# cheneeheng/2s-AGCN

Measured on AMD Instinct MI355X. Metric: skeleton-clips/sec fwd+bwd, NTU (N,3,300,25,2), higher is better.
Workload: dtype f32; 1 GPU; AGCN joint-stream NTU-xview shape, full training step (fwd, CE, bwd, grad all-reduce, clip 1.0, SGD nesterov); per_gpu_batch=64, global_batch=64, input=(N,3,300,25,2), parallelism=dp1, bn=per-replica

## Files before the change

### 2s-agcn_amd/csrc/conv_gemm_bf16.hip

```cpp
#include "agcn_common.h"
#include "epilogue.h"
#include "gate.h"
#include "split_f16.h"

namespace {

typedef __bf16 bf16x8 __attribute__((ext_vector_type(8)));
typedef __bf16 bf16x2 __attribute__((ext_vector_type(2)));
typedef float f32x2 __attribute__((ext_vector_type(2)));
typedef unsigned u32x4 __attribute__((ext_vector_type(4)));
typedef f32x4 f32x4_u __attribute__((aligned(4)));

constexpr int CK = 16, NW = 8, NT = 512;

struct BfArgs {
  const float* in;
  const unsigned short* wp;
  const float* bias;
  float* out;
  float* stats;
  const float* add1;
  const float* mask1;
  const float* add2;
  const float* mask2;
  int N, M, Kinner, in_rows;
  int V, T_src, T_out, tt, ntiles;
  int src_stride, f_off;
  int out_fs, out_fo, T_full;
  int FW, WLR;
  int accumulate;
  int nchunks, nmb;
  int off_b;
  int off_bias;
  int dbg;
  int relu;
  const float* in_absmax;
};

struct GateBfArgs : BfArgs {
  GateArgs gate;
  int off_gate;
};
template <bool GATE> struct BfArgsOf { typedef BfArgs type; };
template <> struct BfArgsOf<true> { typedef GateBfArgs type; };

struct BfPackArgs {
  const float* w;
  unsigned short* wp;
  int M, Kinner, nchunks;
  long sa_m, sa_c;
  int tap_mul, tap_add, tap_flip_from;
};

__device__ __forceinline__ unsigned pack_bf16(float a, float b) {
  f32x2 v = {a, b};
  bf16x2 p = __builtin_convertvector(v, bf16x2);
  return __builtin_bit_cast(unsigned, p);
}
__device__ __forceinline__ float lo_as_f32(unsigned p) { return __builtin_bit_cast(float, p << 16); }
__device__ __forceinline__ float hi_as_f32(unsigned p) { return __builtin_bit_cast(float, p & 0xffff0000u); }

__device__ __forceinline__ void split_pair(float a, float b, unsigned& ph, unsigned& pm, unsigned& pl) {
  ph = pack_bf16(a, b);
  const float ra = a - lo_as_f32(ph), rb = b - hi_as_f32(ph);
  pm = pack_bf16(ra, rb);
  pl = pack_bf16(ra - lo_as_f32(pm), rb - hi_as_f32(pm));
}

template <bool F16>
__device__ __forceinline__ f32x16 mfma_split(bf16x8 x, bf16x8 y, f32x16 c) {
  if constexpr (F16)
    return __builtin_amdgcn_mfma_f32_32x32x16_f16(__builtin_bit_cast(f16x8, x), __builtin_bit_cast(f16x8, y), c, 0, 0, 0);
  else
    return __builtin_amdgcn_mfma_f32_32x32x16_bf16(x, y, c, 0, 0, 0);
}

template <int TAPS, int BM, bool F16 = false>
__global__ void __launch_bounds__(256) pack_weights_bf16_kernel(const BfPackArgs p) {
  constexpr int PER_PLANE = TAPS * 2 * BM * 8;
  const int ch = blockIdx.x % p.nchunks, mb = blockIdx.x / p.nchunks;
  unsigned short* dst = p.wp + (long)blockIdx.x * 3 * PER_PLANE;
  for (int e = threadIdx.x; e < PER_PLANE / 2; e += 256) {
    const int j = (e & 3) * 2;
    const int ml = (e >> 2) % BM;
    const int r = (e >> 2) / BM;
    const int h = r & 1, tap = r >> 1;
    const int m = mb * BM + ml;
    const int gt = p.tap_flip_from >= 0 ? (p.tap_flip_from - (tap * p.tap_mul + p.tap_add)) : tap;
    float v[2];
#pragma unroll
    for (int q = 0; q < 2; ++q) {
      const int kc = ch * CK + h * 8 + j + q;
      v[q] = (m < p.M && kc < p.Kinner) ? p.w[(long)m * p.sa_m + (long)kc * p.sa_c + gt] : 0.f;
    }
    unsigned ph, pm, pl = 0;
    if constexpr (F16) split_pair_f16(v[0] * F16_W_SCALE, v[1] * F16_W_SCALE, ph, pm);
    else split_pair(v[0], v[1], ph, pm, pl);
    const int o = ((tap * 2 + h) * BM + ml) * 8 + j;
    *reinterpret_cast<unsigned*>(dst + 0 * PER_PLANE + o) = ph;
    *reinterpret_cast<unsigned*>(dst + 1 * PER_PLANE + o) = pm;
    *reinterpret_cast<unsigned*>(dst + 2 * PER_PLANE + o) = pl;
  }
}

template <int TAPS, int NPL, int WQ, int TM, int TN = 1, bool F16 = false, bool GATE = false>
__global__ void __launch_bounds__(NT, (TAPS == 1 && TM == 2 && TN == 1) ? 4 : 2) conv_gemm_bf16_kernel(const typename BfArgsOf<GATE>::type a) {
  constexpr int BM = TM * 32;
  constexpr int A_PLANE = TAPS * 2 * BM * 16;
  constexpr int A4 = NPL * A_PLANE / 16;
  constexpr int EA = (A4 + NT - 1) / NT;
  extern __shared__ __attribute__((aligned(16))) unsigned char smem[];
  unsigned char* Ab = smem;
  unsigned char* Bb = smem + a.off_b;

  const int tid = threadIdx.x, lane = tid & 63;
  const int wave = __builtin_amdgcn_readfirstlane(tid >> 6);
  const int lr = lane & 31, h = lane >> 5;
  const int bid = xcd_remap(blockIdx.x, gridDim.x);
  const int mbk = bid % a.nmb;
  const int nt_id = bid / a.nmb;
  const int n = nt_id / a.ntiles, tile_id = nt_id - n * a.ntiles;
  const int m0 = mbk * BM;
  const int V = a.V, tt = a.tt, t0 = tile_id * tt;
  const int ttv = tt * V;
  const int nvalid = min(tt, a.T_out - t0) * V;
  const int Psrc = a.T_src * V;
  const int f0 = t0 * a.src_stride + a.f_off;
  const int WL = a.FW * V, WLR = a.WLR;
  const int g0 = f0 * V;
  float rs_s = 1.f, rs_inv = 1.f;
  if constexpr (F16) { f16_range_scale(a.in_absmax, rs_s, rs_inv); rs_inv *= F16_W_INV; }

  int boff[TN];
#pragma unroll
  for (int tn = 0; tn < TN; ++tn) {
    int q = (wave * TN + tn) * 32 + lr;
    if (q >= ttv) q = 0;
    const int tl = q / V;
    boff[tn] = tl * a.src_stride * V + (q - tl * V);
  }

  float* bias_s = reinterpret_cast<float*>(smem + a.off_bias);
  for (int e = tid; e < BM; e += NT) bias_s[e] = (a.bias && m0 + e < a.M) ? a.bias[m0 + e] : 0.f;

  f32x16 acc[TM][TN];
#pragma unroll
  for (int tm = 0; tm < TM; ++tm)
#pragma unroll
    for (int tn = 0; tn < TN; ++tn)
#pragma unroll
      for (int j = 0; j < 16; ++j) acc[tm][tn][j] = 0.f;

  const int hb = wave & 1, wq = wave >> 1;
  const int qlen = (WL + 3) >> 2;
  u32x4 ra[EA];
  float rb[WQ][8];
  const int KP = a.nchunks * CK;
  const float* gl = nullptr;
  float gpos[WQ];
  if constexpr (GATE) {
    gl = reinterpret_cast<const float*>(smem + a.off_gate);
    gate_stage<NT>(reinterpret_cast<float*>(smem + a.off_gate), a.gate, n, V, a.T_src, a.Kinner, f0, a.FW, KP);
    __syncthreads();
#pragma unroll
    for (int u = 0; u < WQ; ++u) {
      const int rr = lane + 64 * u;
      gpos[u] = rr < qlen ? gate_pos(gl, KP, wq * qlen + rr, V, WL) : 0.f;
    }
    if constexpr (F16) {
      if (a.in_absmax) {
        f16_range_scale_of<14>(*a.in_absmax * gate_bound(gl, KP, a.FW, lane), rs_s, rs_inv);
        rs_inv *= F16_W_INV;
      }
    }
  }
  const u32x4* wp4 = reinterpret_cast<const u32x4*>(a.wp) + (long)mbk * a.nchunks * (3 * A_PLANE / 16);

  auto issue_loads = [&](int ch) __attribute__((always_inline)) {
    const u32x4* src = wp4 + (long)ch * (3 * A_PLANE / 16);
#pragma unroll
    for (int u = 0; u < EA; ++u) ra[u] = src[min(tid + u * NT, A4 - 1)];
    const int kc0 = ch * CK + hb * 8;
#pragma unroll
    for (int u = 0; u < WQ; ++u) {
      const int rr = lane + 64 * u;
      const int r = wq * qlen + rr;
      const int gp = g0 + r;
      const bool okp = rr < qlen && r < WL && gp >= 0 && gp < Psrc;
#pragma unroll
      for (int c = 0; c < 8; ++c) {
        const bool ok = okp && (kc0 + c) < a.Kinner;
        rb[u][c] = a.in[((long)n * a.in_rows + (ok ? (kc0 + c) : 0)) * Psrc + (ok ? gp : 0)];
      }
    }
  };
  auto commit_lds = [&](int ch) __attribute__((always_inline)) {
#pragma unroll
    for (int u = 0; u < EA; ++u)
      if (tid + u * NT < A4) reinterpret_cast<u32x4*>(Ab)[tid + u * NT] = ra[u];
    const int kc0 = ch * CK + hb * 8;
#pragma unroll
    for (int u = 0; u < WQ; ++u) {
      const int rr = lane + 64 * u;
      const int r = wq * qlen + rr;
      const int gp = g0 + r;
      const bool okp = rr < qlen && r < WL && gp >= 0 && gp < Psrc;
      u32x4 ph, pm, pl;
#pragma unroll
      for (int c = 0; c < 4; ++c) {
        float x0 = (okp && (kc0 + 2 * c) < a.Kinner) ? rb[u][2 * c] : 0.f;
        float x1 = (okp && (kc0 + 2 * c + 1) < a.Kinner) ? rb[u][2 * c + 1] : 0.f;
        if constexpr (GATE) {
          x0 = x0 * gpos[u] * gl[kc0 + 2 * c];
          x1 = x1 * gpos[u] * gl[kc0 + 2 * c + 1];
        }
        unsigned a0, a1, a2 = 0;
        if constexpr (F16) split_pair_f16(x0 * rs_s, x1 * rs_s, a0, a1);
        else split_pair(x0, x1, a0, a1, a2);
        ph[c] = a0; pm[c] = a1; pl[c] = a2;
      }
      if (rr < qlen && r < WL) {
        *reinterpret_cast<u32x4*>(Bb + ((0 * 2 + hb) * WLR + r) * 16) = ph;
        if (NPL >= 2) *reinterpret_cast<u32x4*>(Bb + ((1 * 2 + hb) * WLR + r) * 16) = pm;
        if (NPL == 3) *reinterpret_cast<u32x4*>(Bb + ((2 * 2 + hb) * WLR + r) * 16) = pl;
      }
    }
  };

  const int nchunks = a.nchunks;
  if (nchunks > 0) issue_loads(0);
  for (int ch = 0; ch < nchunks; ++ch) {
    __syncthreads();
    if (!(a.dbg & 2) || ch == 0) {
      commit_lds(ch);
      if (ch + 1 < nchunks) issue_loads(ch + 1);
    }
    __syncthreads();
    if (a.dbg & 1) continue;
    bf16x8 afc[NPL], bfc[NPL][TN];
    auto load_a = [&](bf16x8 (&af)[NPL], int tap, int tm) __attribute__((always_inline)) {
#pragma unroll
      for (int pl = 0; pl < NPL; ++pl)
        af[pl] = *reinterpret_cast<const bf16x8*>(Ab + pl * A_PLANE + (((tap * 2 + h) * BM) + tm * 32 + lr) * 16);
    };
    auto load_b = [&](bf16x8 (&bf)[NPL][TN], int tap) __attribute__((always_inline)) {
#pragma unroll
      for (int pl = 0; pl < NPL; ++pl)
#pragma unroll
        for (int tn = 0; tn < TN; ++tn)
          bf[pl][tn] = *reinterpret_cast<const bf16x8*>(Bb + ((pl * 2 + h) * WLR + boff[tn] + tap * V) * 16);
    };
    load_b(bfc, 0);
    load_a(afc, 0, 0);
    __builtin_amdgcn_sched_group_barrier(0x100, NPL * (TN + 1), 0);
#pragma unroll 1
    for (int tap = 0; tap < TAPS; ++tap) {
      bf16x8 bfn[NPL][TN];
      const int tapn = min(tap + 1, TAPS - 1);
#pragma unroll
      for (int tm = 0; tm < TM; ++tm) {
        bf16x8 afn[NPL];
        load_a(afn, tm + 1 == TM ? tapn : tap, tm + 1 == TM ? 0 : tm + 1);
        if (tm + 1 == TM) load_b(bfn, tapn);
#pragma unroll
        for (int tn = 0; tn < TN; ++tn) {
          if (NPL == 3) {
            acc[tm][tn] = mfma_split<F16>(afc[NPL - 1], bfc[0][tn], acc[tm][tn]);
            acc[tm][tn] = mfma_split<F16>(afc[0], bfc[NPL - 1][tn], acc[tm][tn]);
            acc[tm][tn] = mfma_split<F16>(afc[NPL >= 2 ? 1 : 0], bfc[NPL >= 2 ? 1 : 0][tn], acc[tm][tn]);
          }
          if (NPL >= 2) {
            acc[tm][tn] = mfma_split<F16>(afc[NPL >= 2 ? 1 : 0], bfc[0][tn], acc[tm][tn]);
            acc[tm][tn] = mfma_split<F16>(afc[0], bfc[NPL >= 2 ? 1 : 0][tn], acc[tm][tn]);
          }
          acc[tm][tn] = mfma_split<F16>(afc[0], bfc[0][tn], acc[tm][tn]);
        }
        __builtin_amdgcn_sched_group_barrier(0x100, NPL, 0);
        if (tm + 1 == TM) __builtin_amdgcn_sched_group_barrier(0x100, NPL * TN, 0);
        __builtin_amdgcn_sched_group_barrier(0x008, TN * (NPL == 3 ? 6 : NPL == 2 ? 3 : 1), 0);
#pragma unroll
        for (int pl = 0; pl < NPL; ++pl) afc[pl] = afn[pl];
      }
#pragma unroll
      for (int pl = 0; pl < NPL; ++pl)
#pragma unroll
        for (int tn = 0; tn < TN; ++tn) bfc[pl][tn] = bfn[pl][tn];
    }
  }

  if ((a.dbg & 4) && acc[0][0][0] != 12345.f) return;
  __syncthreads();
  float* tile = reinterpret_cast<float*>(smem);
  const int TP = NW * TN * 32 + 1;
  float* red = tile + BM * TP;
#pragma unroll
  for (int tm = 0; tm < TM; ++tm)
#pragma unroll
    for (int tn = 0; tn < TN; ++tn)
#pragma unroll
      for (int j = 0; j < 16; ++j)
        tile[(tm * 32 + mfma_row(j, h)) * TP + (wave * TN + tn) * 32 + lr] = F16 ? acc[tm][tn][j] * rs_inv : acc[tm][tn][j];
  __syncthreads();
  int poff[4 * TN];
#pragma unroll
  for (int u = 0; u < 4 * TN; ++u) {
    const int q2 = lane + 64 * u;
    const int tl2 = q2 / V;
    poff[u] = tl2 * a.out_fs * V + (q2 - tl2 * V);
  }
  EpiPtrs ep;
  ep.out = a.out; ep.add1 = a.add1; ep.mask1 = a.mask1; ep.add2 = a.add2; ep.mask2 = a.mask2; ep.stats = a.stats;
  ep.accumulate = a.accumulate; ep.relu = a.relu;
  const long Pfull = (long)a.T_full * V;
  const long rows0 = (long)n * a.M * Pfull + ((long)t0 * a.out_fs + a.out_fo) * V;
  epilogue_rows<BM, NW, 4 * TN>(ep, tile, TP, bias_s, red, a.M, m0, rows0, Pfull, nvalid, poff, (long)n * a.ntiles + tile_id);
}


template <int TAPS, int NPL, int R, int NWP = 4, bool F16 = false, bool GATE = false>
__global__ void __launch_bounds__((8 + NWP) * 64, 3) conv_pc_kernel(const typename BfArgsOf<GATE>::type a) {
  constexpr int TM = 4, BM = 128, NWC = 8, NTALL = (NWC + NWP) * 64, NTP = NWP * 64;
  constexpr int SLOT = NPL * 2 * BM * 16;
  constexpr int PIECES = SLOT / 1024;
  constexpr int PPW = (PIECES + NWP - 1) / NWP;
  constexpr int NMF = NPL == 3 ? 6 : NPL == 2 ? 3 : 1;
  extern __shared__ __attribute__((aligned(16))) unsigned char smem[];
  unsigned char* ring = smem;
  const int WLR = a.WLR, V = a.V;
  const int B_BYTES = NPL * 2 * WLR * 16;
  unsigned char* Bbase = smem + a.off_b;

  const int wave = __builtin_amdgcn_readfirstlane(threadIdx.x >> 6);
  const int lane = threadIdx.x & 63;
  const int bid = xcd_remap(blockIdx.x, gridDim.x);
  const int mbk = bid % a.nmb;
  const int nt_id = bid / a.nmb;
  const int n = nt_id / a.ntiles, tile_id = nt_id - n * a.ntiles;
  const int m0 = mbk * BM;
  const int tt = a.tt, t0 = tile_id * tt;
  const int ttv = tt * V;
  const int nvalid = min(tt, a.T_out - t0) * V;
  const int Psrc = a.T_src * V;
  const int g0 = (t0 + a.f_off) * V;
  const int WL = a.FW * V;
  const int nchunks = a.nchunks;
  const int G = nchunks * TAPS;
  float rs_s = 1.f, rs_inv = 1.f;
  if constexpr (F16) { f16_range_scale(a.in_absmax, rs_s, rs_inv); rs_inv *= F16_W_INV; }

  float* bias_s = reinterpret_cast<float*>(smem + a.off_bias);
  for (int e = threadIdx.x; e < BM; e += NTALL) bias_s[e] = (a.bias && m0 + e < a.M) ? a.bias[m0 + e] : 0.f;
  const int KP = nchunks * CK;
  const float* gl = nullptr;
  if constexpr (GATE) {
    gl = reinterpret_cast<const float*>(smem + a.off_gate);
    gate_stage<NTALL>(reinterpret_cast<float*>(smem + a.off_gate), a.gate, n, V, a.T_src, a.Kinner, t0 + a.f_off, a.FW, KP);
    __syncthreads();
    if constexpr (F16) {
      if (a.in_absmax) {
        f16_range_scale_of<14>(*a.in_absmax * gate_bound(gl, KP, a.FW, lane), rs_s, rs_inv);
        rs_inv *= F16_W_INV;
      }
    }
  }

  auto step_barrier = [&]() __attribute__((always_inline)) {
    asm volatile("s_waitcnt lgkmcnt(0)\n\ts_barrier" ::: "memory");
  };

  if (wave >= NWC) {
    const int pw = wave - NWC;
    typedef const __attribute__((address_space(1))) void* gptr_t;
    typedef __attribute__((address_space(3))) void* lptr_t;
    const unsigned char* wsrc = reinterpret_cast<const unsigned char*>(a.wp) + (long)mbk * G * SLOT + lane * 16;
    auto dma_slot = [&](int g) __attribute__((always_inline)) {
      const unsigned char* src = wsrc + (long)g * SLOT;
      unsigned char* dst = ring + (g % R) * SLOT;
#pragma unroll
      for (int u = 0; u < PPW; ++u) {
        const int piece = pw + u * NWP;
        if (piece < PIECES)
          __builtin_amdgcn_global_load_lds((gptr_t)(src + piece * 1024), (lptr_t)(dst + piece * 1024), 16, 0, 0);
      }
    };
    const int ptid = threadIdx.x - NWC * 64;
    const int npiece = (WL + 3) >> 2;
    const int ntask = 2 * npiece;
    constexpr int TK = 256 / NTP;
    f32x4 rb[TK][8];
    auto issue_B = [&](int ch) __attribute__((always_inline)) {
#pragma unroll
      for (int k = 0; k < TK; ++k) {
        if (k * NTP >= ntask) continue;
        int task = ptid + k * NTP;
        if (task >= ntask) task = ntask - 1;
        const int hb = task & 1, r0 = (task >> 1) * 4;
        const int gp = g0 + r0;
        const float* src = a.in + ((long)n * a.in_rows + ch * CK + hb * 8) * Psrc + gp;
        if (gp >= 0 && gp + 3 < Psrc) {
#pragma unroll
          for (int c = 0; c < 8; ++c) rb[k][c] = *reinterpret_cast<const f32x4_u*>(src + (long)c * Psrc);
        } else {
#pragma unroll
          for (int c = 0; c < 8; ++c)
#pragma unroll
            for (int e = 0; e < 4; ++e) {
              const bool ok = gp + e >= 0 && gp + e < Psrc;
              const float t = src[(long)c * Psrc + (ok ? e : -gp)];
              rb[k][c][e] = ok ? t : 0.f;
            }
        }
      }
    };
    float gpos[TK][4];
    if constexpr (GATE) {
#pragma unroll
      for (int k = 0; k < TK; ++k) {
        int task = ptid + k * NTP;
        if (task >= ntask) task = ntask - 1;
#pragma unroll
        for (int e = 0; e < 4; ++e) gpos[k][e] = (k * NTP < ntask) ? gate_pos(gl, KP, (task >> 1) * 4 + e, V, WL) : 0.f;
      }
    }
    auto commit_B = [&](unsigned char* Bb, int ch) __attribute__((always_inline)) {
#pragma unroll
      for (int k = 0; k < TK; ++k) {
        if (k * NTP >= ntask) continue;
        int task = ptid + k * NTP;
        if (task >= ntask) task = ntask - 1;
        const int hb = task & 1, r0 = (task >> 1) * 4;
        float gch[8];
        if constexpr (GATE) {
          const f32x4 g0v = *reinterpret_cast<const f32x4*>(gl + ch * CK + hb * 8);
          const f32x4 g1v = *reinterpret_cast<const f32x4*>(gl + ch * CK + hb * 8 + 4);
#pragma unroll
          for (int c = 0; c < 4; ++c) { gch[c] = g0v[c]; gch[4 + c] = g1v[c]; }
        }
#pragma unroll
        for (int e = 0; e < 4; ++e) {
          u32x4 ph, pm, pl;
#pragma unroll
          for (int c = 0; c < 4; ++c) {
            unsigned q0, q1, q2 = 0;
            float x0 = rb[k][2 * c][e], x1 = rb[k][2 * c + 1][e];
            if constexpr (GATE) {
              x0 = x0 * gpos[k][e] * gch[2 * c];
              x1 = x1 * gpos[k][e] * gch[2 * c + 1];
            }
            if constexpr (F16) split_pair_f16(x0 * rs_s, x1 * rs_s, q0, q1);
            else split_pair(x0, x1, q0, q1, q2);
            ph[c] = q0; pm[c] = q1; pl[c] = q2;
          }
          const int r = r0 + e;
          if (r < WLR) {
            *reinterpret_cast<u32x4*>(Bb + ((0 * 2 + hb) * WLR + r) * 16) = ph;
            if (NPL >= 2) *reinterpret_cast<u32x4*>(Bb + ((1 * 2 + hb) * WLR + r) * 16) = pm;
            if (NPL == 3) *reinterpret_cast<u32x4*>(Bb + ((2 * 2 + hb) * WLR + r) * 16) = pl;
          }
        }
      }
    };
#pragma unroll
    for (int g = 0; g < R - 1; ++g)
      if (g < G) dma_slot(g);
    issue_B(0);
    commit_B(Bbase, 0);
    asm volatile("s_waitcnt vmcnt(0)" ::: "memory");
    step_barrier();
    int g = 0;
    for (int ch = 0; ch < nchunks; ++ch) {
#pragma unroll
      for (int tap = 0; tap < TAPS; ++tap, ++g) {
        if (a.dbg & 2) { step_barrier(); continue; }
        if (g + R - 1 < G && !(a.dbg & 8)) dma_slot(g + R - 1);
        if (TAPS >= 3) {
          if (tap == 0 && ch + 1 < nchunks && !(a.dbg & 4)) issue_B(ch + 1);
          if (tap == (TAPS >= 6 ? TAPS - 3 : TAPS - 2) && ch + 1 < nchunks && !(a.dbg & 4))
            commit_B(Bbase + ((ch + 1) & 1) * B_BYTES, ch + 1);
        } else {
          if (tap == 0 && ch + 1 < nchunks) { issue_B(ch + 1); commit_B(Bbase + ((ch + 1) & 1) * B_BYTES, ch + 1); }
        }
        if (g + R - 1 < G) asm volatile("s_waitcnt vmcnt(%0)" :: "n"(PPW * (R - 3)) : "memory");
        else asm volatile("s_waitcnt vmcnt(0)" ::: "memory");
        step_barrier();
      }
    }
    return;
  }

  const int lr = lane & 31, h = lane >> 5;
  int q = wave * 32 + lr;
  if (q >= ttv) q = 0;
  const int boff = q;
  f32x16 acc[TM];
#pragma unroll
  for (int tm = 0; tm < TM; ++tm)
#pragma unroll
    for (int j = 0; j < 16; ++j) acc[tm][j] = 0.f;

  const unsigned char* a_lane = ring + (h * BM + lr) * 16;
  auto load_a = [&](bf16x8 (&af)[NPL], int slot, int tm) __attribute__((always_inline)) {
#pragma unroll
    for (int pl = 0; pl < NPL; ++pl)
      af[pl] = *reinterpret_cast<const bf16x8*>(a_lane + slot * SLOT + (pl * 2 * BM + tm * 32) * 16);
  };
  auto load_b = [&](bf16x8 (&bf)[NPL], const unsigned char* Bb, int tap) __attribute__((always_inline)) {
#pragma unroll
    for (int pl = 0; pl < NPL; ++pl)
      bf[pl] = *reinterpret_cast<const bf16x8*>(Bb + ((pl * 2 + h) * WLR + boff + tap * V) * 16);
  };
  step_barrier();
  bf16x8 afc[NPL], bfc[NPL];
  load_b(bfc, Bbase, 0);
  load_a(afc, 0, 0);
  int slot = 0;
  for (int ch = 0; ch < nchunks; ++ch) {
    const unsigned char* Bb = Bbase + (ch & 1) * B_BYTES;
    const unsigned char* Bn = Bbase + ((ch + 1) & 1) * B_BYTES;
#pragma unroll
    for (int tap = 0; tap < TAPS; ++tap) {
      const int slot_n = (slot + 1 == R) ? 0 : slot + 1;
      if (a.dbg & 1) { step_barrier(); continue; }
      bf16x8 bfn[NPL];
#pragma unroll
      for (int tm = 0; tm < TM; ++tm) {
        bf16x8 afn[NPL];
        if (tm + 1 < TM) {
          load_a(afn, slot, tm + 1);
        } else {
          load_a(afn, slot_n, 0);
          if (tap + 1 < TAPS) load_b(bfn, Bb, tap + 1);
          else load_b(bfn, Bn, 0);
        }
        if (NPL == 3) {
          acc[tm] = mfma_split<F16>(afc[NPL - 1], bfc[0], acc[tm]);
          acc[tm] = mfma_split<F16>(afc[0], bfc[NPL - 1], acc[tm]);
          acc[tm] = mfma_split<F16>(afc[NPL >= 2 ? 1 : 0], bfc[NPL >= 2 ? 1 : 0], acc[tm]);
        }
        if (NPL >= 2) {
          acc[tm] = mfma_split<F16>(afc[NPL >= 2 ? 1 : 0], bfc[0], acc[tm]);
          acc[tm] = mfma_split<F16>(afc[0], bfc[NPL >= 2 ? 1 : 0], acc[tm]);
        }
        acc[tm] = mfma_split<F16>(afc[0], bfc[0], acc[tm]);
        __builtin_amdgcn_sched_group_barrier(0x100, NPL, 0);
        if (tm + 1 == TM) __builtin_amdgcn_sched_group_barrier(0x100, NPL, 0);
        __builtin_amdgcn_sched_group_barrier(0x008, NMF, 0);
#pragma unroll
        for (int pl = 0; pl < NPL; ++pl) afc[pl] = afn[pl];
      }
#pragma unroll
      for (int pl = 0; pl < NPL; ++pl) bfc[pl] = bfn[pl];
      slot = slot_n;
      step_barrier();
    }
  }

  float* tile = reinterpret_cast<float*>(smem);
  const int TP = NWC * 32 + 1;
  float* red = tile + BM * TP;
#pragma unroll
  for (int tm = 0; tm < TM; ++tm)
#pragma unroll
    for (int j = 0; j < 16; ++j) tile[(tm * 32 + mfma_row(j, h)) * TP + wave * 32 + lr] = F16 ? acc[tm][j] * rs_inv : acc[tm][j];
  __syncthreads();
  int poff[4];
#pragma unroll
  for (int u = 0; u < 4; ++u) {
    const int q2 = lane + 64 * u;
    const int tl2 = q2 / V;
    poff[u] = tl2 * a.out_fs * V + (q2 - tl2 * V);
  }
  EpiPtrs ep;
  ep.out = a.out; ep.add1 = a.add1; ep.mask1 = a.mask1; ep.add2 = a.add2; ep.mask2 = a.mask2; ep.stats = a.stats;
  ep.accumulate = a.accumulate; ep.relu = a.relu;
  const long Pfull = (long)a.T_full * V;
  const long rows0 = (long)n * a.M * Pfull + ((long)t0 * a.out_fs + a.out_fo) * V;
  epilogue_rows<BM, NWC, 4>(ep, tile, TP, bias_s, red, a.M, m0, rows0, Pfull, nvalid, poff, (long)n * a.ntiles + tile_id);
}

template <int TAPS, int BM, int NPL, bool F16 = false>
__global__ void __launch_bounds__(256) pack_weights_slots_kernel(const BfPackArgs p) {
  constexpr int PLANE = 2 * BM * 8;
  const int tap = blockIdx.x % TAPS;
  const int ch = (blockIdx.x / TAPS) % p.nchunks, mb = blockIdx.x / (TAPS * p.nchunks);
  unsigned short* dst = p.wp + (long)blockIdx.x * NPL * PLANE;
  const int gt = p.tap_flip_from >= 0 ? (p.tap_flip_from - (tap * p.tap_mul + p.tap_add)) : tap;
  for (int e = threadIdx.x; e < PLANE / 2; e += 256) {
    const int j = (e & 3) * 2;
    const int ml = (e >> 2) % BM;
    const int h = (e >> 2) / BM;
    const int m = mb * BM + ml;
    float v[2];
#pragma unroll
    for (int q = 0; q < 2; ++q) {
      const int kc = ch * CK + h * 8 + j + q;
      v[q] = (m < p.M && kc < p.Kinner) ? p.w[(long)m * p.sa_m + (long)kc * p.sa_c + gt] : 0.f;
    }
    unsigned ph, pm, pl = 0;
    if constexpr (F16) split_pair_f16(v[0] * F16_W_SCALE, v[1] * F16_W_SCALE, ph, pm);
    else split_pair(v[0], v[1], ph, pm, pl);
    const int o = (h * BM + ml) * 8 + j;
    *reinterpret_cast<unsigned*>(dst + 0 * PLANE + o) = ph;
    if (NPL >= 2) *reinterpret_cast<unsigned*>(dst + 1 * PLANE + o) = pm;
    if (NPL == 3) *reinterpret_cast<unsigned*>(dst + 2 * PLANE + o) = pl;
  }
}

struct BfGeom {
  int tt, ntiles, FW, WLR, nchunks, nmb, off_b, off_bias;
  size_t smem_bytes, pack_bytes;
};

template <int TAPS, int BM, int TN = 1>
BfGeom bf_geometry(int V, int T_out, int src_stride, int M, int Kinner) {
  BfGeom g;
  g.tt = (256 * TN) / V;
  if (g.tt > T_out) g.tt = T_out;
  if (g.tt < 1) g.tt = 1;
  g.ntiles = (T_out + g.tt - 1) / g.tt;
  g.FW = (g.tt - 1) * src_stride + TAPS;
  g.WLR = g.FW * V + 8;
  g.nchunks = (Kinner + CK - 1) / CK;
  g.nmb = (M + BM - 1) / BM;
  const size_t a_bytes = (size_t)3 * TAPS * 2 * BM * 16;
  g.off_b = (int)a_bytes;
  const size_t b_bytes = (size_t)3 * 2 * g.WLR * 16;
  size_t main_b = a_bytes + b_bytes;
  size_t epi_b = (size_t)BM * (NW * TN * 32 + 1) * 4 + (size_t)NT * 2 * 4;
  g.smem_bytes = ((main_b > epi_b ? main_b : epi_b) + 15) & ~(size_t)15;
  g.off_bias = (int)g.smem_bytes;
  g.smem_bytes += (size_t)BM * 4;
  g.pack_bytes = (size_t)g.nmb * g.nchunks * a_bytes;
  return g;
}

struct BfProblem {
  BfArgs a;
  GateArgs gate;
  int fwd_f16;
  const float* w;
  long sa_m, sa_c;
  int tap_mul, tap_add, tap_flip_from;
  void* ws;
  size_t ws_bytes;
  int stats_tiles;
};

inline size_t gate_bytes(const BfGeom& g) { return 4 * (size_t)gate_lds_floats(g.FW, g.nchunks * CK); }

template <int TAPS, int NPL, int WQ, int TM, int TN = 1, bool F16 = false, bool GATE = false>
int launch_bf(BfProblem& p, hipStream_t stream) {
  constexpr int BM = TM * 32;
  typename BfArgsOf<GATE>::type a;
  static_cast<BfArgs&>(a) = p.a;
  BfGeom g = bf_geometry<TAPS, BM, TN>(a.V, a.T_out, a.src_stride, a.M, a.Kinner);
  if constexpr (GATE) {
    a.gate = p.gate;
    a.off_gate = (int)g.smem_bytes;
    g.smem_bytes += gate_bytes(g);
  }
  if (g.smem_bytes > 160 * 1024) return AGCN_ERR_UNSUPPORTED;
  if ((g.FW * a.V + 3) / 4 > WQ * 64) return AGCN_ERR_UNSUPPORTED;
  if (g.pack_bytes > p.ws_bytes) return AGCN_ERR_WORKSPACE;
  if (a.stats && p.stats_tiles > 0 && g.ntiles != p.stats_tiles) return AGCN_ERR_ARG;
  a.tt = g.tt; a.ntiles = g.ntiles; a.FW = g.FW; a.WLR = g.WLR; a.nchunks = g.nchunks; a.nmb = g.nmb;
  a.off_b = g.off_b; a.off_bias = g.off_bias;
  a.wp = (const unsigned short*)p.ws;
  static const int dbg = getenv("AGCN_CB_DBG") ? atoi(getenv("AGCN_CB_DBG")) : 0;
  a.dbg = dbg;
  if (g.nchunks > 0) {
    BfPackArgs pk;
    pk.w = p.w; pk.wp = (unsigned short*)p.ws; pk.M = a.M; pk.Kinner = a.Kinner; pk.nchunks = g.nchunks;
    pk.sa_m = p.sa_m; pk.sa_c = p.sa_c;
    pk.tap_mul = p.tap_mul; pk.tap_add = p.tap_add; pk.tap_flip_from = p.tap_flip_from;
    hipLaunchKernelGGL((pack_weights_bf16_kernel<TAPS, BM, F16>), dim3(g.nmb * g.nchunks), dim3(256), 0, stream, pk);
    int rc = agcn_check_launch();
    if (rc) return rc;
  }
  auto kern = conv_gemm_bf16_kernel<TAPS, NPL, WQ, TM, TN, F16, GATE>;
  static unsigned char lds_ok[AGCN_MAX_DEVICES] = {};
  if (int e = agcn_allow_big_lds_rt(reinterpret_cast<const void*>(kern), lds_ok)) return e;
  if (GATE) AGCN_NOTE_KERNEL("conv_gemm_bf16_kernel<%d, %d, %d, %d, %d, %s, true> [gates on load]", TAPS, NPL, WQ, TM, TN, F16 ? "true" : "false");
  else AGCN_NOTE_KERNEL("conv_gemm_bf16_kernel<%d, %d, %d, %d, %d, %s>", TAPS, NPL, WQ, TM, TN, F16 ? "true" : "false");
  hipLaunchKernelGGL(kern, dim3((unsigned)(a.N * g.ntiles * g.nmb)), dim3(NT), g.smem_bytes, stream, a);
  return agcn_check_launch();
}


template <int TAPS, int NPL, int R>
BfGeom bf_geometry_pc(int V, int T_out, int M, int Kinner) {
  constexpr int BM = 128, SLOT = NPL * 2 * BM * 16;
  BfGeom g;
  g.tt = 256 / V;
  if (g.tt > T_out) g.tt = T_out;
  if (g.tt < 1) g.tt = 1;
  g.ntiles = (T_out + g.tt - 1) / g.tt;
  g.FW = (g.tt - 1) + TAPS;
  g.WLR = g.FW * V + 8;
  g.nchunks = (Kinner + CK - 1) / CK;
  g.nmb = (M + BM - 1) / BM;
  g.off_b = R * SLOT;
  const size_t main_b = (size_t)g.off_b + 2 * (size_t)NPL * 2 * g.WLR * 16;
  const size_t epi_b = (size_t)BM * (8 * 32 + 1) * 4 + (size_t)512 * 2 * 4;
  g.smem_bytes = ((main_b > epi_b ? main_b : epi_b) + 15) & ~(size_t)15;
  g.off_bias = (int)g.smem_bytes;
  g.smem_bytes += (size_t)BM * 4;
  g.pack_bytes = (size_t)g.nmb * g.nchunks * TAPS * SLOT;
  return g;
}

static inline bool conv_pc_enabled() {
  static int v = -1;
  if (v < 0) {
    const char* e = getenv("AGCN_CONV_PC");
    v = (e && atoi(e) == 0) ? 0 : 1;
  }
  return v == 1;
}

template <int TAPS, int NPL, int R = 5, int NWP = 4, bool F16 = false, bool GATE = false>
int launch_pc(BfProblem& p, hipStream_t stream) {
  constexpr int BM = 128;
  typename BfArgsOf<GATE>::type a;
  static_cast<BfArgs&>(a) = p.a;
  BfGeom g = bf_geometry_pc<TAPS, NPL, R>(a.V, a.T_out, a.M, a.Kinner);
  if constexpr (GATE) {
    a.gate = p.gate;
    a.off_gate = (int)g.smem_bytes;
    g.smem_bytes += gate_bytes(g);
  }
  if (g.smem_bytes > 160 * 1024) return AGCN_ERR_UNSUPPORTED;
  if (g.pack_bytes > p.ws_bytes) return AGCN_ERR_WORKSPACE;
  if (a.stats && p.stats_tiles > 0 && g.ntiles != p.stats_tiles) return AGCN_ERR_ARG;
  a.tt = g.tt; a.ntiles = g.ntiles; a.FW = g.FW; a.WLR = g.WLR; a.nchunks = g.nchunks; a.nmb = g.nmb;
  a.off_b = g.off_b; a.off_bias = g.off_bias;
  a.wp = (const unsigned short*)p.ws;
  BfPackArgs pk;
  pk.w = p.w; pk.wp = (unsigned short*)p.ws; pk.M = a.M; pk.Kinner = a.Kinner; pk.nchunks = g.nchunks;
  pk.sa_m = p.sa_m; pk.sa_c = p.sa_c;
  pk.tap_mul = p.tap_mul; pk.tap_add = p.tap_add; pk.tap_flip_from = p.tap_flip_from;
  hipLaunchKernelGGL((pack_weights_slots_kernel<TAPS, BM, NPL, F16>), dim3(g.nmb * g.nchunks * TAPS), dim3(256), 0, stream, pk);
  int rc = agcn_check_launch();
  if (rc) return rc;
  auto kern = conv_pc_kernel<TAPS, NPL, R, NWP, F16, GATE>;
  static unsigned char lds_ok[AGCN_MAX_DEVICES] = {};
  if (int e = agcn_allow_big_lds_rt(reinterpret_cast<const void*>(kern), lds_ok)) return e;
  static const int dbg = getenv("AGCN_CB_DBG") ? atoi(getenv("AGCN_CB_DBG")) : 0;
  a.dbg = dbg;
  if (GATE) AGCN_NOTE_KERNEL("conv_pc_kernel<%d, %d, %d, %d, %s, true> [gates on load]", TAPS, NPL, R, NWP, F16 ? "true" : "false");
  else AGCN_NOTE_KERNEL("conv_pc_kernel<%d, %d, %d, %d, %s>", TAPS, NPL, R, NWP, F16 ? "true" : "false");
  hipLaunchKernelGGL(kern, dim3((unsigned)(a.N * g.ntiles * g.nmb)), dim3((8 + NWP) * 64), g.smem_bytes, stream, a);
  return agcn_check_launch();
}

template <int TAPS>
bool pc_applies(const BfProblem& p, int npl, bool gate = false) {
  if (!conv_pc_enabled() || TAPS < 3 || npl != 3) return false;
  if (p.a.M % 128 != 0 || p.a.Kinner % CK != 0 || p.a.src_stride != 1 || p.a.V > 32) return false;
  const BfGeom g = bf_geometry_pc<TAPS, 3, 5>(p.a.V, p.a.T_out, p.a.M, p.a.Kinner);
  return g.smem_bytes + (gate ? gate_bytes(g) : 0) <= 160 * 1024 && g.FW * p.a.V <= 512;
}

template <int TAPS, int WQ, bool GATE = false>
int launch_npl(BfProblem& p, int npl, hipStream_t s) {
  const BfGeom g128 = bf_geometry<TAPS, 128>(p.a.V, p.a.T_out, p.a.src_stride, p.a.M, p.a.Kinner);
  const bool fits128 = g128.smem_bytes + (GATE ? gate_bytes(g128) : 0) <= 160 * 1024;
  if constexpr (TAPS >= 3) {
    if (pc_applies<TAPS>(p, npl, GATE)) {
      static const int nwp2 = getenv("AGCN_CONV_NWP2") ? atoi(getenv("AGCN_CONV_NWP2")) : 0;
      if (nwp2 && !GATE) return launch_pc<TAPS, 3, 5, 2>(p, s);
      if (p.fwd_f16) return launch_pc<TAPS, 2, 5, 4, true, GATE>(p, s);
      return launch_pc<TAPS, 3, 5, 4, false, GATE>(p, s);
    }
  }
  if constexpr (TAPS >= 3) {
    if (p.fwd_f16) {
      if (p.a.M % 128 == 0 && fits128) return launch_bf<TAPS, 2, WQ, 4, 1, true, GATE>(p, s);
      if (agcn_bf16_conv_wide(TAPS, p.a.M)) {
        const int rc = launch_bf<TAPS, 2, 3, 2, 2, true, GATE>(p, s);
        if (rc != AGCN_ERR_UNSUPPORTED) return rc;
      }
      return launch_bf<TAPS, 2, WQ, 2, 1, true, GATE>(p, s);
    }
  }
  if (p.a.M % 128 == 0 && fits128) {
    if (npl == 1) return launch_bf<TAPS, 1, WQ, 4, 1, false, GATE>(p, s);
    return npl == 2 ? launch_bf<TAPS, 2, WQ, 4, 1, false, GATE>(p, s) : launch_bf<TAPS, 3, WQ, 4, 1, false, GATE>(p, s);
  }
  if (agcn_bf16_conv_wide(TAPS, p.a.M) && (npl == 3 || npl == 1)) {
    const int rc = npl == 3 ? launch_bf<TAPS, 3, 3, 2, 2, false, GATE>(p, s) : launch_bf<TAPS, 1, 3, 2, 2, false, GATE>(p, s);
    if (rc != AGCN_ERR_UNSUPPORTED) return rc;
  }
  if (npl == 1) return launch_bf<TAPS, 1, WQ, 2, 1, false, GATE>(p, s);
  return npl == 2 ? launch_bf<TAPS, 2, WQ, 2, 1, false, GATE>(p, s) : launch_bf<TAPS, 3, WQ, 2, 1, false, GATE>(p, s);
}

}

bool agcn_bf16_conv_wide(int taps, int M) {
  static int v = -1;
  if (v < 0) {
    const char* e = getenv("AGCN_CONV_WIDE");
    v = (e && atoi(e) == 0) ? 0 : 1;
  }
  return v == 1 && taps > 1 && M <= 64;
}

size_t agcn_bf16_conv_workspace(int Cin, int Cout, int T, int V, int stride) {
  const int To = (T + 8 - 9) / stride + 1;
  size_t b = bf_geometry<9, 64>(V, To, stride, Cout, Cin).pack_bytes, t;
  t = bf_geometry<9, 64>(V, T, 1, Cin, Cout).pack_bytes; if (t > b) b = t;
  t = bf_geometry<9, 128>(V, To, stride, Cout, Cin).pack_bytes; if (t > b) b = t;
  t = bf_geometry<9, 128>(V, T, 1, Cin, Cout).pack_bytes; if (t > b) b = t;
  return b + 256;
}

namespace {

int bf16_in_absmax(BfProblem& p, const float* given, const float* in, long n, hipStream_t s) {
  if (given) {
    p.a.in_absmax = given;
    return 0;
  }
  if (p.ws_bytes < 64) return AGCN_ERR_WORKSPACE;
  unsigned* amax = reinterpret_cast<unsigned*>(static_cast<char*>(p.ws) + ((p.ws_bytes - 16) & ~(size_t)15));
  if (hipMemsetAsync(amax, 0, 4, s) != hipSuccess) return AGCN_ERR_ARG;
  hipLaunchKernelGGL(absmax_kernel, dim3(2048), dim3(256), 0, s, in, n, amax);
  if (int rc = agcn_check_launch()) return rc;
  p.a.in_absmax = reinterpret_cast<const float*>(amax);
  p.ws_bytes = (p.ws_bytes - 16) & ~(size_t)15;
  return 0;
}

int bf16_fwd_f16x3(int npl) {
  static const int f16x3 = getenv("AGCN_CONV_F16X3") ? atoi(getenv("AGCN_CONV_F16X3")) : 1;
  return f16x3 && npl == 3;
}

template <int TAPS, int WQ, bool GATE = false>
int bf16_tconv_fwd(const float* x, const float* w, const float* bias, float* y, float* stats_part, void* ws,
                   size_t ws_bytes, int N, int Cin, int Cout, int T, int V, int stride, int pad, int npl, hipStream_t s,
                   const float* add, int relu, const float* x_absmax, const GateArgs* gate = nullptr) {
  BfProblem p = {};
  BfArgs& a = p.a;
  a.in = x; a.bias = bias; a.out = y; a.stats = stats_part; a.add1 = add; a.relu = relu;
  if (GATE) p.gate = *gate;
  p.fwd_f16 = bf16_fwd_f16x3(npl);
  p.ws = ws; p.ws_bytes = ws_bytes;
  if (p.fwd_f16)
    if (int rc = bf16_in_absmax(p, x_absmax, x, (long)N * Cin * T * V, s)) return rc;
  a.N = N; a.M = Cout; a.Kinner = Cin; a.in_rows = Cin; a.V = V;
  a.T_src = T; a.T_out = (T + 2 * pad - TAPS) / stride + 1; a.T_full = a.T_out;
  a.src_stride = stride; a.f_off = -pad; a.out_fs = 1; a.out_fo = 0;
  p.w = w; p.sa_m = (long)Cin * TAPS; p.sa_c = TAPS; p.tap_flip_from = -1;
  if (TAPS != 9 && stats_part) {
    const int tt = agcn_bf16_tconv_tile_frames(TAPS, Cout, V, a.T_out, npl);
    p.stats_tiles = (a.T_out + tt - 1) / tt;
  }
  return launch_npl<TAPS, WQ, GATE>(p, npl, s);
}

template <int TAPS>
int bf16_tconv_bwd_data_s1(const float* dy, const float* w, float* dx, int accumulate, const float* add1,
                           const float* mask1, const float* add2, const float* mask2, void* ws, size_t ws_bytes, int N,
                           int Cin, int Cout, int T, int V, int pad, int npl, hipStream_t s, const float* dy_absmax) {
  BfProblem p = {};
  BfArgs& a = p.a;
  p.fwd_f16 = bf16_fwd_f16x3(npl);
  p.ws = ws; p.ws_bytes = ws_bytes;
  const int To = T + 2 * pad - TAPS + 1;
  if (p.fwd_f16)
    if (int rc = bf16_in_absmax(p, dy_absmax, dy, (long)N * Cout * To * V, s)) return rc;
  a.in = dy; a.out = dx; a.accumulate = accumulate;
  a.add1 = add1; a.mask1 = mask1; a.add2 = add2; a.mask2 = mask2;
  a.N = N; a.M = Cin; a.Kinner = Cout; a.in_rows = Cout; a.V = V;
  a.T_src = To; a.T_full = T; a.src_stride = 1;
  a.T_out = T; a.out_fs = 1; a.out_fo = 0; a.f_off = pad - (TAPS - 1);
  p.w = w; p.sa_m = TAPS; p.sa_c = (long)Cin * TAPS;
  p.tap_mul = 1; p.tap_add = 0; p.tap_flip_from = TAPS - 1;
  return launch_npl<TAPS, 2>(p, npl, s);
}

}

int agcn_bf16_conv9_fwd(const float* x, const float* w, const float* bias, float* y, float* stats_part, void* ws,
                        size_t ws_bytes, int N, int Cin, int Cout, int T, int V, int stride, int npl,
                        hipStream_t s, const float* add, int relu, const float* x_absmax) {
  if (stride == 1)
    return bf16_tconv_fwd<9, 2>(x, w, bias, y, stats_part, ws, ws_bytes, N, Cin, Cout, T, V, 1, 4, npl, s, add, relu,
                                x_absmax);
  return bf16_tconv_fwd<9, 3>(x, w, bias, y, stats_part, ws, ws_bytes, N, Cin, Cout, T, V, stride, 4, npl, s, add, relu,
                              x_absmax);
}

int agcn_bf16_conv9_bwd_data(const float* dy, const float* w, float* dx, int accumulate, const float* add1,
                             const float* mask1, const float* add2, const float* mask2, void* ws, size_t ws_bytes,
                             int N, int Cin, int Cout, int T, int V, int stride, int npl, hipStream_t s,
                             const float* dy_absmax) {
  if (stride == 1)
    return bf16_tconv_bwd_data_s1<9>(dy, w, dx, accumulate, add1, mask1, add2, mask2, ws, ws_bytes, N, Cin, Cout, T, V,
                                     4, npl, s, dy_absmax);
  BfProblem p = {};
  BfArgs& a = p.a;
  p.fwd_f16 = bf16_fwd_f16x3(npl);
  p.ws = ws; p.ws_bytes = ws_bytes;
  if (p.fwd_f16)
    if (int rc = bf16_in_absmax(p, dy_absmax, dy, (long)N * Cout * ((T + 8 - 9) / stride + 1) * V, s)) return rc;
  a.in = dy; a.out = dx; a.accumulate = accumulate;
  a.add1 = add1; a.mask1 = mask1; a.add2 = add2; a.mask2 = mask2;
  a.N = N; a.M = Cin; a.Kinner = Cout; a.in_rows = Cout; a.V = V;
  a.T_src = (T + 8 - 9) / stride + 1; a.T_full = T; a.src_stride = 1;
  p.w = w; p.sa_m = 9; p.sa_c = (long)Cin * 9;
  a.T_out = (T + 1) / 2; a.out_fs = 2; a.out_fo = 0; a.f_off = -2;
  p.tap_mul = 2; p.tap_add = 0; p.tap_flip_from = 8;
  int rc = launch_npl<5, 2>(p, npl, s);
  if (rc) return rc;
  a.T_out = T / 2; a.out_fo = 1; a.f_off = -1;
  p.tap_add = 1;
  if (a.T_out > 0) rc = launch_npl<4, 2>(p, npl, s);
  return rc;
}

bool agcn_bf16_tconv_supported(int taps, int stride) { return stride == 1 && (taps == 3 || taps == 5 || taps == 7); }

int agcn_bf16_tconv_fwd(const float* x, const float* w, const float* bias, float* y, float* stats_part, void* ws,
                        size_t ws_bytes, int N, int Cin, int Cout, int T, int V, int taps, int pad, int npl,
                        hipStream_t s, const float* x_absmax) {
  switch (taps) {
    case 3: return bf16_tconv_fwd<3, 2>(x, w, bias, y, stats_part, ws, ws_bytes, N, Cin, Cout, T, V, 1, pad, npl, s,
                                        nullptr, 0, x_absmax);
    case 5: return bf16_tconv_fwd<5, 2>(x, w, bias, y, stats_part, ws, ws_bytes, N, Cin, Cout, T, V, 1, pad, npl, s,
                                        nullptr, 0, x_absmax);
    case 7: return bf16_tconv_fwd<7, 2>(x, w, bias, y, stats_part, ws, ws_bytes, N, Cin, Cout, T, V, 1, pad, npl, s,
                                        nullptr, 0, x_absmax);
    default: return AGCN_ERR_UNSUPPORTED;
  }
}

int agcn_bf16_tconv_bwd_data(const float* dy, const float* w, float* dx, int accumulate, const float* add1,
                             const float* mask1, const float* add2, const float* mask2, void* ws, size_t ws_bytes,
                             int N, int Cin, int Cout, int T, int V, int taps, int pad, int npl, hipStream_t s,
                             const float* dy_absmax) {
  switch (taps) {
    case 3: return bf16_tconv_bwd_data_s1<3>(dy, w, dx, accumulate, add1, mask1, add2, mask2, ws, ws_bytes, N, Cin, Cout,
                                             T, V, pad, npl, s, dy_absmax);
    case 5: return bf16_tconv_bwd_data_s1<5>(dy, w, dx, accumulate, add1, mask1, add2, mask2, ws, ws_bytes, N, Cin, Cout,
                                             T, V, pad, npl, s, dy_absmax);
    case 7: return bf16_tconv_bwd_data_s1<7>(dy, w, dx, accumulate, add1, mask1, add2, mask2, ws, ws_bytes, N, Cin, Cout,
                                             T, V, pad, npl, s, dy_absmax);
    default: return AGCN_ERR_UNSUPPORTED;
  }
}

template <int TAPS, int WQ>
static int bf16_tconv_infer_t(const float* x, const float* w, const float* bias, float* y, void* ws, size_t ws_bytes, int N,
                              int Cin, int Cout, int T, int V, int stride, int pad, int npl, hipStream_t s,
                              const float* add, int relu, const float* x_absmax, const GateArgs* gate) {
  const bool gated = gate && (gate->gs || gate->gt || gate->gc);
  {
    const int To = (T + 2 * pad - TAPS) / stride + 1;
    const BfGeom g = bf_geometry<TAPS, 64>(V, To, stride, Cout, Cin);
    if (g.smem_bytes + (gated ? gate_bytes(g) : 0) > 160 * 1024 || (g.FW * V + 3) / 4 > WQ * 64) return AGCN_ERR_UNSUPPORTED;
  }
  if (gated)
    return bf16_tconv_fwd<TAPS, WQ, true>(x, w, bias, y, nullptr, ws, ws_bytes, N, Cin, Cout, T, V, stride, pad, npl, s, add,
                                          relu, x_absmax, gate);
  return bf16_tconv_fwd<TAPS, WQ>(x, w, bias, y, nullptr, ws, ws_bytes, N, Cin, Cout, T, V, stride, pad, npl, s, add, relu,
                                  x_absmax);
}

bool agcn_bf16_tconv_infer_supported(int taps, int stride, int pad) {
  if (taps == 9) return pad == 4 && (stride == 1 || stride == 2);
  return agcn_bf16_tconv_supported(taps, stride);
}

int agcn_bf16_tconv_infer(const float* x, const float* w, const float* bias, float* y, void* ws, size_t ws_bytes, int N,
                          int Cin, int Cout, int T, int V, int taps, int stride, int pad, int npl, hipStream_t s,
                          const float* add, int relu, const float* x_absmax, const GateArgs* gate) {
  if (!agcn_bf16_tconv_infer_supported(taps, stride, pad)) return AGCN_ERR_UNSUPPORTED;
#define AGCN_INFER_CASE(TAPS, WQ) \
  return bf16_tconv_infer_t<TAPS, WQ>(x, w, bias, y, ws, ws_bytes, N, Cin, Cout, T, V, stride, pad, npl, s, add, relu, x_absmax, gate)
  switch (taps) {
    case 3: AGCN_INFER_CASE(3, 2);
    case 5: AGCN_INFER_CASE(5, 2);
    case 7: AGCN_INFER_CASE(7, 2);
    default: break;
  }
  if (stride == 1) AGCN_INFER_CASE(9, 2);
  AGCN_INFER_CASE(9, 3);
#undef AGCN_INFER_CASE
}

int agcn_bf16_tconv_tile_frames(int taps, int M, int V, int T_out, int npl) {
  int tt = 256 / V;
  if (M <= 64 && agcn_bf16_conv_wide(taps, M) && (npl == 3 || npl == 1)) {
    bool ok = false;
    switch (taps) {
      case 3: ok = bf_geometry<3, 64, 2>(V, T_out, 1, M, 16).smem_bytes <= 160 * 1024; break;
      case 5: ok = bf_geometry<5, 64, 2>(V, T_out, 1, M, 16).smem_bytes <= 160 * 1024; break;
      case 7: ok = bf_geometry<7, 64, 2>(V, T_out, 1, M, 16).smem_bytes <= 160 * 1024; break;
      default: break;
    }
    int tw = 512 / V;
    if (tw > T_out) tw = T_out;
    if (ok && ((tw - 1) + taps) * V <= 3 * 64 * 4) tt = 512 / V;
  }
  if (tt > T_out) tt = T_out;
  if (tt < 1) tt = 1;
  return tt;
}

int agcn_bf16_conv1_fwd(const float* x, const float* w, const float* bias, float* y, float* stats_part, void* ws,
                        size_t ws_bytes, int N, int Cin, int Cout, int T, int V, int stride, int npl,
                        hipStream_t s, const float* add, int relu) {
  BfProblem p = {};
  BfArgs& a = p.a;
  a.in = x; a.bias = bias; a.out = y; a.stats = stats_part; a.add1 = add; a.relu = relu;
  a.N = N; a.M = Cout; a.Kinner = Cin; a.in_rows = Cin; a.V = V;
  a.T_src = T; a.T_out = (T - 1) / stride + 1; a.T_full = a.T_out;
  a.src_stride = stride; a.f_off = 0; a.out_fs = 1; a.out_fo = 0;
  p.w = w; p.sa_m = Cin; p.sa_c = 1; p.tap_flip_from = -1;
  p.ws = ws; p.ws_bytes = ws_bytes;
  if (stride == 1) return launch_npl<1, 2>(p, npl, s);
  return launch_npl<1, 3>(p, npl, s);
}

int agcn_bf16_conv1_bwd_data(const float* dy, const float* w, float* dx, int accumulate, const float* add1,
                             const float* mask1, const float* add2, const float* mask2, void* ws, size_t ws_bytes,
                             int N, int Cin, int Cout, int T, int V, int npl, hipStream_t s) {
  BfProblem p = {};
  BfArgs& a = p.a;
  a.in = dy; a.out = dx; a.accumulate = accumulate;
  a.add1 = add1; a.mask1 = mask1; a.add2 = add2; a.mask2 = mask2;
  a.N = N; a.M = Cin; a.Kinner = Cout; a.in_rows = Cout; a.V = V;
  a.T_src = T; a.T_full = T; a.src_stride = 1;
  a.T_out = T; a.out_fs = 1; a.out_fo = 0; a.f_off = 0;
  p.w = w; p.sa_m = 1; p.sa_c = Cin; p.tap_mul = 1; p.tap_add = 0; p.tap_flip_from = 0;
  p.ws = ws; p.ws_bytes = ws_bytes;
  return launch_npl<1, 2>(p, npl, s);
}

size_t agcn_bf16_conv1_workspace(int Cin, int Cout, int T, int V, int stride) {
  const int To = (T - 1) / stride + 1;
  size_t b = bf_geometry<1, 64>(V, To, stride, Cout, Cin).pack_bytes, t;
  t = bf_geometry<1, 64>(V, T, 1, Cin, Cout).pack_bytes; if (t > b) b = t;
  t = bf_geometry<1, 128>(V, To, stride, Cout, Cin).pack_bytes; if (t > b) b = t;
  t = bf_geometry<1, 128>(V, T, 1, Cin, Cout).pack_bytes; if (t > b) b = t;
  return b + 256;
}
```

### 2s-agcn_amd/csrc/epilogue.h

```cpp
#pragma once
#include "agcn_common.h"

struct EpiPtrs {
  float* out;
  const float* add1;
  const float* mask1;
  const float* add2;
  const float* mask2;
  float* stats;
  int accumulate;
  int relu;
};

template <int BM, int NW, int XB>
__device__ __forceinline__ void epilogue_rows(const EpiPtrs& e, const float* tile, int TP, const float* bias_s,
                                              float* red, int M, int m0, long rows0, long P, int nvalid,
                                              const int (&poff)[XB], long stats_slot) {
  constexpr int NT = NW * 64;
  const int tid = threadIdx.x, lane = tid & 63;
  const int wave = __builtin_amdgcn_readfirstlane(tid >> 6);
  constexpr int RG = (XB >= 8) ? 1 : ((XB >= 4) ? 2 : 4), NG = BM / (NW * RG);
  static_assert(BM % (NW * RG) == 0, "row groups must tile the block");
  const bool has_extra = e.accumulate || e.add1 || e.add2;
  float ex[2][5][RG][XB];
  auto row_base = [&](int k, int g) __attribute__((always_inline)) {
    const int m = min(m0 + (k * NW + wave) * RG + g, M - 1);
    return rows0 + (long)m * P;
  };
  auto load_extras = [&](int k, float (&x)[5][RG][XB]) __attribute__((always_inline)) {
#pragma unroll
    for (int g = 0; g < RG; ++g) {
      const long base = row_base(k, g);
#pragma unroll
      for (int u = 0; u < XB; ++u) {
        const int q = lane + 64 * u;
        const long idx = base + ((q < nvalid) ? poff[u] : 0);
        if (e.accumulate) x[0][g][u] = e.out[idx];
        if (e.add1) x[1][g][u] = e.add1[idx];
        if (e.mask1) x[2][g][u] = e.mask1[idx];
        if (e.add2) x[3][g][u] = e.add2[idx];
        if (e.mask2) x[4][g][u] = e.mask2[idx];
      }
    }
  };
  if (has_extra) load_extras(0, ex[0]);
  if (e.stats) {
    constexpr int NP = NT / BM;
    static_assert(NT % BM == 0, "threads must tile the rows");
    const int r = tid % BM, part = tid / BM;
    const float bval = bias_s[r];
    float bsum = 0.f, bsq = 0.f;
#pragma unroll 8
    for (int q = part; q < nvalid; q += NP) {
      const float y = tile[r * TP + q] + bval;
      bsum += y;
      bsq += y * y;
    }
    red[(part * 2 + 0) * BM + r] = bsum;
    red[(part * 2 + 1) * BM + r] = bsq;
    __syncthreads();
    for (int i = tid; i < 2 * BM; i += NT) {
      const int k = i / BM, ml = i - k * BM;
      float sum = 0.f;
#pragma unroll
      for (int p2 = 0; p2 < NP; ++p2) sum += red[(p2 * 2 + k) * BM + ml];
      if (m0 + ml < M) e.stats[(stats_slot * 2 + k) * M + m0 + ml] = sum;
    }
  }
#pragma unroll
  for (int k = 0; k < NG; ++k) {
    const int r0 = (k * NW + wave) * RG;
    if (m0 + r0 >= M) break;
    if (has_extra && k + 1 < NG) load_extras(k + 1, ex[(k + 1) & 1]);
#pragma unroll
    for (int g = 0; g < RG; ++g) {
      const int m = m0 + r0 + g;
      if (m >= M) break;
      const long base = row_base(k, g);
      const float bval = bias_s[r0 + g];
#pragma unroll
      for (int u = 0; u < XB; ++u) {
        const int q = lane + 64 * u;
        float v = tile[(r0 + g) * TP + min(q, TP - 1)] + bval;
        if (e.accumulate) v += ex[k & 1][0][g][u];
        if (e.add1) v += (!e.mask1 || ex[k & 1][2][g][u] > 0.f) ? ex[k & 1][1][g][u] : 0.f;
        if (e.add2) v += (!e.mask2 || ex[k & 1][4][g][u] > 0.f) ? ex[k & 1][3][g][u] : 0.f;
        if (e.relu) v = fmaxf(v, 0.f);
        if (q < nvalid) e.out[base + poff[u]] = v;
      }
    }
  }
}
```

### 2s-agcn_amd/lib.py

```python
import ctypes
import os

import torch

_HERE = os.path.dirname(os.path.abspath(__file__))
LIB_PATH = os.path.join(_HERE, "libagcn_hip.so")

_P = ctypes.c_void_p
_I = ctypes.c_int
_F = ctypes.c_float
_D = ctypes.c_double
_Z = ctypes.c_size_t

SIGNATURES = {
    "agcn_version": (_I, []),
    "agcn_arch": (ctypes.c_char_p, []),
    "agcn_last_kernel": (ctypes.c_char_p, []),
    "agcn_gemm_mode": (ctypes.c_char_p, []),
    "agcn_chain_mode": (ctypes.c_char_p, []),
    "agcn_conv_tile_frames": (_I, [_I, _I]),
    "agcn_conv_num_tiles": (_I, [_I, _I]),
    "agcn_conv_stats_tiles": (_I, [_I, _I, _I, _I, _I, _I]),
    "agcn_dadj_num_slots": (_I, [_I, _I, _I]),
    "agcn_scores_num_tiles": (_I, [_I, _I]),
    "agcn_conv_workspace": (_Z, [_I, _I, _I, _I, _I, _I]),
    "agcn_gcn_workspace": (_Z, [_I, _I, _I, _I]),
    "agcn_gcn_stats_tiles": (_I, [_I, _I, _I, _I]),
    "agcn_gcn_stats_slots": (_I, [_I, _I, _I, _I, _I]),
    "agcn_conv_fwd": (_I, [_P, _P, _P, _P, _P, _P, _Z, _I, _I, _I, _I, _I, _I, _I, _P]),
    "agcn_conv_bwd_data": (_I, [_P, _P, _P, _I, _P, _P, _P, _P, _P, _Z, _I, _I, _I, _I, _I, _I, _I, _P]),
    "agcn_conv_bwd_weight_workspace": (_Z, [_I, _I, _I, _I, _I, _I, _I]),
    "agcn_conv_bwd_weight": (_I, [_P, _P, _P, _P, _Z, _I, _I, _I, _I, _I, _I, _I, _P]),
    "agcn_gcn_aggregate_project_fwd": (_I, [_P, _P, _P, _P, _P, _P, _P, _Z, _I, _I, _I, _I, _I, _P]),
    "agcn_gcn_aggregate_project_fwd_ex": (_I, [_P, _P, _P, _P, _P, _P, _P, _Z, _I, _I, _I, _I, _I, _P, _P]),
    "agcn_gcn_aggregate_project_bwd_data_ex": (_I, [_P, _P, _P, _P, _P, _I, _P, _I, _P, _P, _P, _P, _I, _P, _Z, _I, _I, _I, _I, _I, _P, _P, _P]),
    "agcn_gcn_dadj_ex": (_I, [_P, _P, _P, _P, _P, _Z, _I, _I, _I, _I, _I, _P, _P, _P]),
    "agcn_adjacency_bwd_scores_ex": (_I, [_P, _P, _P, _P, _P, _P, _P, _I, _I, _I, _I, _P]),
    "agcn_conv_bwd_weight_ex": (_I, [_P, _P, _P, _P, _Z, _I, _I, _I, _I, _I, _I, _I, _P, _P, _P]),
    "agcn_gcn_project_bwd_weight_ex": (_I, [_P, _P, _P, _P, _P, _Z, _I, _I, _I, _I, _I, _P, _P, _P]),
    "agcn_absmax": (_I, [_P, ctypes.c_long, _P, _P]),
    "agcn_tconv_workspace": (_Z, [_I] * 7),
    "agcn_tconv_stats_tiles": (_I, [_I] * 7),
    "agcn_tconv_fwd": (_I, [_P] * 6 + [_Z] + [_I] * 8 + [_P, _P]),
    "agcn_tconv_bwd_data": (_I, [_P, _P, _P, _I, _P, _P, _P, _P, _P, _Z] + [_I] * 8 + [_P, _P]),
    "agcn_tconv_bwd_weight_workspace": (_Z, [_I] * 8),
    "agcn_tconv_bwd_weight": (_I, [_P] * 4 + [_Z] + [_I] * 8 + [_P] * 3),
    "agcn_bn_act_fwd_ex": (_I, [_P, _P, _P, _P, _P, _P, _P, _P, _P, _I, _I, _I, _I, _I, _P]),
    "agcn_bn_bwd_apply_ex": (_I, [_P, _I, _D, _F, _P, _P, _I] + [_P] * 16 + [_I, _I, _I, _P]),
    "agcn_conv_fwd_ex": (_I, [_P, _P, _P, _P, _P, _P, _Z, _I, _I, _I, _I, _I, _I, _I, _P, _P]),
    "agcn_conv_bwd_data_ex": (_I, [_P, _P, _P, _I, _P, _P, _P, _P, _P, _Z, _I, _I, _I, _I, _I, _I, _I, _P, _P]),
    "agcn_gcn_first_supported": (_I, [_I, _I, _I]),
    "agcn_gcn_first_tiles": (_I, [_I, _I]),
    "agcn_gcn_first_fwd": (_I, [_P, _P, _P, _P, _P, _P, _P, _P, _P, _P, _I, _I, _I, _I, _I, _P]),
    "agcn_gcn_unit_infer_workspace": (_Z, [_I, _I, _I, _I, _I]),
    "agcn_gcn_unit_infer": (_I, [_P, _P, _P, _P, _P, _P, _P, _I, _I, _P, _P, _Z, _I, _I, _I, _I, _I, _P]),
    "agcn_conv9_infer": (_I, [_P, _P, _P, _P, _I, _P, _P, _Z, _I, _I, _I, _I, _I, _I, _P]),
    "agcn_tconv_infer": (_I, [_P] * 7 + [_I, _P, _P, _Z] + [_I] * 8 + [_P, _P]),
    "agcn_gcn_aggregate_project_bwd_data": (_I, [_P, _P, _P, _P, _I, _P, _P, _P, _P, _I, _P, _Z, _I, _I, _I, _I, _I, _P]),
    "agcn_gcn_bwd_data_fused_supported": (_I, [_I, _I, _I]),
    "agcn_gcn_aggregate_project_bwd_data_fused": (_I, [_P, _P, _P, _P, _P, _I, _P, _I, _P, _P, _P, _P, _I, _P, _Z, _I, _I, _I, _I, _I, _P]),
    "agcn_gcn_dadj": (_I, [_P, _P, _P, _P, _P, _Z, _I, _I, _I, _I, _I, _P]),
    "agcn_gcn_project_bwd_weight_workspace": (_Z, [_I, _I, _I, _I, _I]),
    "agcn_gcn_project_bwd_weight": (_I, [_P, _P, _P, _P, _P, _Z, _I, _I, _I, _I, _I, _P]),
    "agcn_adjacency_fwd": (_I, [_P, _P, _P, _P, _P, _P, _P, _I, _I, _I, _I, _P]),
    "agcn_adjacency_fused_supported": (_I, [_I, _I, _I, _I]),
    "agcn_adjacency_fused_workspace": (_Z, [_I, _I]),
    "agcn_adjacency_fused_fwd": (_I, [_P, _P, _P, _P, _P, _P, _P, _P, _P, _P, _P, _Z, _I, _I, _I, _I, _I, _P]),
    "agcn_adjacency_fused_fwd_ex": (_I, [_P, _P, _P, _P, _P, _P, _P, _P, _P, _P, _P, _P, _P, _Z, _I, _I, _I, _I, _I, _P]),
    "agcn_adjacency_fused_bwd_scores": (_I, [_P, _P, _P, _P, _P, _P, _P, _P, _P, _Z, _I, _I, _I, _I, _I, _P]),
    "agcn_adjacency_bwd_softmax": (_I, [_P, _P, _P, _P, _P, _P, _P, _I, _I, _I, _I, _I, _P]),
    "agcn_adjacency_bwd_scores": (_I, [_P, _P, _P, _P, _P, _P, _I, _I, _I, _I, _P]),
    "agcn_colsum_scratch_bytes": (_Z, [_I]),
    "agcn_colsum": (_I, [_P, _I, _I, _P, _P, _P]),
    "agcn_bn_stats_finalize": (_I, [_P, _I, _I, _D, _P, _P, _P, _P, _F, _F, _P, _P, _P, _P, _P, _P]),
    "agcn_bn_eval_coeff": (_I, [_P, _P, _P, _P, _F, _I, _P, _P, _P]),
    "agcn_bn_act_fwd": (_I, [_P, _P, _P, _P, _P, _P, _P, _P, _I, _I, _I, _I, _I, _P]),
    "agcn_bn_bwd": (_I, [_P, _P, _I] + [_P] * 16 + [_I, _I, _I, _P]),
    "agcn_bn_bwd_reduce": (_I, [_P, _P, _I, _P, _P, _P, _I, _I, _I, _P]),
    "agcn_bn_bwd_apply": (_I, [_P, _I, _D, _F, _P, _P, _I] + [_P] * 15 + [_I, _I, _I, _P]),
    "agcn_bn_eval_coeff_ex": (_I, [_P, _P, _P, _P, _F, _I, _P, _P, _P, _P, _P]),
    "agcn_bn_bwd_eval": (_I, [_P, _P, _I, _P, _P, _P, _P, _I, _P, _P, _P, _P, _I, _I, _I, _P]),
    "agcn_bn_bwd_eval_finalize": (_I, [_P, _I, _I] + [_P] * 13),
    "agcn_stc_row_reduce": (_I, [_P, _P, _P, _P, _I, _P, _P, _F, _F, _I, _I, _I, _I, _P]),
    "agcn_stc_apply": (_I, [_P, _P, _P, _P, _P, _I, _I, _I, _I, _P]),
    "agcn_stc_apply_ex": (_I, [_P, _P, _P, _P, _P, _P, _I, _I, _I, _I, _P]),
    "agcn_stc_bwd_apply": (_I, [_P, _P, _P, _P, _P, _P, _P, _I, _I, _I, _I, _P]),
    "agcn_data_bn_stats": (_I, [_P, _P, _I, _I, _I, _I, _I, _P]),
    "agcn_data_bn_apply": (_I, [_P, _P, _P, _P, _I, _I, _I, _I, _I, _P]),
    "agcn_data_bn_bwd_reduce": (_I, [_P, _P, _P, _P, _P, _I, _I, _I, _I, _I, _P]),
    "agcn_data_bn_bwd_apply": (_I, [_P, _P, _P, _P, _P, _P, _D, _P, _I, _I, _I, _I, _I, _P]),
    "agcn_pool_fwd": (_I, [_P, _P, _P, _I, _I, _I, _I, _P]),
    "agcn_pool_bwd": (_I, [_P, _P, _I, _I, _I, _I, _P]),
    "agcn_linear_fwd": (_I, [_P, _P, _P, _P, _I, _I, _I, _I, _P]),
    "agcn_linear_bwd": (_I, [_P, _P, _P, _P, _P, _P, _P, _P, _I, _I, _I, _I, _P]),
    "agcn_gate_conv_fwd": (_I, [_P, _P, _P, _P, _I, _I, _I, _I, _P]),
    "agcn_gate_conv_bwd": (_I, [_P, _P, _P, _P, _P, _P, _P, _P, _I, _I, _I, _I, _P]),
    "agcn_sgd_step_workspace": (_Z, [ctypes.c_long]),
    "agcn_sgd_step": (_I, [_P, _P, _P, ctypes.c_long, _F, _F, _F, _I, _F, _F, _I, _P, _Z, _P, _P]),
}

_lib = None


def load():
    global _lib
    if _lib is not None:
        return _lib
    if not os.path.exists(LIB_PATH):
        raise RuntimeError(
            f"agcn_amd: HIP extension {LIB_PATH} not found -- run `python -c 'import __graft_entry__ as g; "
            f"g.build()'` (hipcc --offload-arch=gfx950).  There is no CPU fallback for the hot path.")
    lib = ctypes.CDLL(LIB_PATH)
    for name, (res, args) in SIGNATURES.items():
        fn = getattr(lib, name)
        fn.restype = res
        fn.argtypes = args
    _lib = lib
    return lib


def ptr_bits(t):
    if t is None:
        return None
    if not (t.is_cuda and t.is_contiguous() and t.dtype == torch.int32):
        raise RuntimeError(f"agcn_amd: expected a contiguous int32 GPU tensor, got {t.dtype} on {t.device}")
    return t.data_ptr()


def ptr(t):
    if t is None:
        return None
    if not (t.is_cuda and t.is_contiguous() and t.dtype == torch.float32):
        raise RuntimeError(f"agcn_amd: expected a contiguous fp32 GPU tensor, got {t.dtype} "
                           f"{tuple(t.shape)} on {t.device} contiguous={t.is_contiguous()}")
    return t.data_ptr()


def stream():
    return torch.cuda.current_stream().cuda_stream


def check(rc, what):
    if rc != 0:
        raise RuntimeError(f"agcn_amd: {what} failed with code {rc}")
```

### 2s-agcn_amd/ops.py

```python
import os
import weakref

import torch

from . import lib as _lib

BN_EPS = 1e-5
BN_MOMENTUM = 0.1


def _L():
    return _lib.load()


def _empty(shape, like):
    return torch.empty(shape, dtype=torch.float32, device=like.device)


def _ws(nbytes, like):
    return torch.empty((int(nbytes) + 3) // 4, dtype=torch.float32, device=like.device)


def _conv_ws(Cin, Cout, T, V, taps, stride, like, pad=None):
    pad = (taps - 1) // 2 if pad is None else pad
    n = _L().agcn_tconv_workspace(Cin, Cout, T, V, taps, stride, pad)
    return _ws(n, like), n


def _gcn_ws(C, Cout, T, V, like):
    n = _L().agcn_gcn_workspace(C, Cout, T, V)
    return _ws(n, like), n


def _scratch(width, like):
    nbytes = _L().agcn_colsum_scratch_bytes(int(width))
    return torch.empty((nbytes + 7) // 8, dtype=torch.float64, device=like.device)



_SIDE = {}


def side_stream_enabled():
    return os.environ.get('AGCN_SIDE_STREAM', '1') != '0'


_SIDE_SCOPE = [0]


def _side_run(fn, inputs):
    if not side_stream_enabled() or _SIDE_SCOPE[0] <= 0:
        return fn()
    main = torch.cuda.current_stream()
    dev = main.device_index
    side = _SIDE.get(dev)
    if side is None:
        side = _SIDE[dev] = torch.cuda.Stream(device=dev)
    side.wait_stream(main)
    with torch.cuda.stream(side):
        out = fn()
    for t in inputs:
        if t is not None:
            t.record_stream(side)
    outs = out if isinstance(out, (tuple, list)) else (out,)
    for t in outs:
        if torch.is_tensor(t):
            t.record_stream(main)
    return out


def _side_join():
    if side_stream_enabled():
        main = torch.cuda.current_stream()
        side = _SIDE.get(main.device_index)
        if side is not None:
            main.wait_stream(side)


def fused_amax_enabled():
    return os.environ.get('AGCN_FUSED_AMAX', '1') != '0'


_OUT_AMAX = [None]
_OUT_AMAX_STATS = [0, 0]


def _note_out_amax(t, amax):
    _OUT_AMAX[0] = (weakref.ref(t), t._version, amax) if amax is not None else None


def _take_out_amax(t):
    e = _OUT_AMAX[0]
    hit = e is not None and e[0]() is t and t._version == e[1]
    _OUT_AMAX_STATS[int(hit)] += 1
    return e[2] if hit else None


def conv_out_frames(T, taps, stride, pad=None):
    pad = (taps - 1) // 2 if pad is None else pad
    return (T + 2 * pad - taps) // stride + 1


def conv_fwd(x, w, b, stride=1, want_stats=False, x_amax=None, pad=None):
    N, Cin, T, V = x.shape
    Cout, Cin2, taps, one = w.shape
    assert Cin2 == Cin and one == 1
    pad = (taps - 1) // 2 if pad is None else pad
    To = conv_out_frames(T, taps, stride, pad)
    if To < 1:
        raise ValueError(f"agcn_amd: a {taps}-frame kernel with padding {pad} does not fit {T} frames")
    y = _empty((N, Cout, To, V), x)
    stats = None
    if want_stats:
        nt = _L().agcn_tconv_stats_tiles(Cin, Cout, To, V, taps, stride, pad)
        stats = _empty((N * nt, 2, Cout), x)
    ws, nb = _conv_ws(Cin, Cout, T, V, taps, stride, x, pad)
    _lib.check(_L().agcn_tconv_fwd(_lib.ptr(x), _lib.ptr(w), _lib.ptr(b), _lib.ptr(y), _lib.ptr(stats), ws.data_ptr(),
                                   nb, N, Cin, Cout, T, V, taps, stride, pad, _lib.ptr(x_amax), _lib.stream()),
               "agcn_tconv_fwd")
    return y, stats


def conv_bwd_data(dy, w, x_shape, stride=1, out=None, accumulate=False, add1=None, mask1=None, add2=None,
                  mask2=None, dy_amax=None, pad=None):
    N, Cin, T, V = x_shape
    Cout, _, taps, _ = w.shape
    pad = (taps - 1) // 2 if pad is None else pad
    dx = out if out is not None else _empty(x_shape, dy)
    ws, nb = _conv_ws(Cin, Cout, T, V, taps, stride, dy, pad)
    _lib.check(_L().agcn_tconv_bwd_data(_lib.ptr(dy), _lib.ptr(w), _lib.ptr(dx), int(accumulate), _lib.ptr(add1),
                                        _lib.ptr(mask1), _lib.ptr(add2), _lib.ptr(mask2), ws.data_ptr(), nb, N, Cin,
                                        Cout, T, V, taps, stride, pad, _lib.ptr(dy_amax), _lib.stream()),
               "agcn_tconv_bwd_data")
    return dx


def conv_bwd_weight(dy, x, w_shape, stride=1, dy_amax=None, x_amax=None, pad=None):
    N, Cin, T, V = x.shape
    Cout, _, taps, _ = w_shape
    pad = (taps - 1) // 2 if pad is None else pad
    nbytes = _L().agcn_tconv_bwd_weight_workspace(N, Cin, Cout, T, V, taps, stride, pad)
    ws = torch.empty((nbytes + 3) // 4, dtype=torch.float32, device=x.device)
    dw = _empty(tuple(w_shape), x)
    _lib.check(_L().agcn_tconv_bwd_weight(_lib.ptr(dy), _lib.ptr(x), _lib.ptr(dw), _lib.ptr(ws), nbytes, N, Cin, Cout,
                                          T, V, taps, stride, pad, _lib.ptr(dy_amax), _lib.ptr(x_amax), _lib.stream()),
               "agcn_tconv_bwd_weight")
    return dw


def adjacency_fwd(tp, A, PA, alpha=None):
    N, C6, T, V = tp.shape
    Ci = C6 // 6
    nt = _L().agcn_scores_num_tiles(V, T)
    spart = _empty((N, 3, nt, V, V), tp)
    P = _empty((N, 3, V, V), tp)
    adj = _empty((N, 3, V, V), tp)
    _lib.check(_L().agcn_adjacency_fwd(_lib.ptr(tp), _lib.ptr(A), _lib.ptr(PA), _lib.ptr(alpha), _lib.ptr(spart),
                                       _lib.ptr(P), _lib.ptr(adj), N, Ci, T, V, _lib.stream()), "agcn_adjacency_fwd")
    return P, adj


def adjacency_fused_supported(C, Ci, T, V):
    return bool(_L().agcn_adjacency_fused_supported(int(C), int(Ci), int(T), int(V)))


def adjacency_recompute():
    import os
    return os.environ.get('AGCN_ADJ_RECOMPUTE', '0') == '1'


def adjacency_fused_fwd(x, wab, bab, A, PA, alpha=None, keep_tp=False, x_amax_out=None, x_amax=None):
    N, C, T, V = x.shape
    Ci = wab.shape[0] // 6
    tp = _empty((N, 6 * Ci, T, V), x) if keep_tp else None
    nt = _L().agcn_scores_num_tiles(V, T)
    spart = _empty((N, 3, nt, V, V), x)
    P = _empty((N, 3, V, V), x)
    adj = _empty((N, 3, V, V), x)
    nb = _L().agcn_adjacency_fused_workspace(C, Ci)
    ws = _ws(nb, x)
    _lib.check(_L().agcn_adjacency_fused_fwd_ex(_lib.ptr(x), _lib.ptr(wab.reshape(6 * Ci, C)), _lib.ptr(bab), _lib.ptr(A),
                                                _lib.ptr(PA), _lib.ptr(alpha), _lib.ptr(tp), _lib.ptr(spart), _lib.ptr(P),
                                                _lib.ptr(adj), _lib.ptr(x_amax_out), _lib.ptr(x_amax), ws.data_ptr(), nb, N,
                                                C, Ci, T, V, _lib.stream()), "agcn_adjacency_fused_fwd")
    return (P, adj, tp) if keep_tp else (P, adj)


def first_layer_enabled():
    return os.environ.get('AGCN_FIRST_LAYER', '1') != '0'


def gcn_first_fwd(x, adj, wcat, bias, wdown, bdown, want_stats=False):
    N, C, T, V = x.shape
    Cout = wcat.shape[0]
    ypre, dpre = _empty((N, Cout, T, V), x), _empty((N, Cout, T, V), x)
    st = st2 = None
    if want_stats:
        nt = _L().agcn_gcn_first_tiles(T, V)
        st, st2 = _empty((N * nt, 2, Cout), x), _empty((N * nt, 2, Cout), x)
    wdown2 = wdown.reshape(Cout, C).contiguous()
    _lib.check(_L().agcn_gcn_first_fwd(_lib.ptr(x), _lib.ptr(adj), _lib.ptr(wcat), _lib.ptr(bias), _lib.ptr(wdown2),
                                       _lib.ptr(bdown), _lib.ptr(ypre), _lib.ptr(st), _lib.ptr(dpre), _lib.ptr(st2),
                                       N, C, Cout, T, V, _lib.stream()), "agcn_gcn_first_fwd")
    return ypre, st, dpre, st2


def aggregate_project_fwd(x, adj, wcat, bias, want_stats=False, x_amax=None):
    N, C, T, V = x.shape
    Cout = wcat.shape[0]
    y = _empty((N, Cout, T, V), x)
    stats = None
    if want_stats:
        stats = _empty((_L().agcn_gcn_stats_slots(N, C, Cout, T, V), 2, Cout), x)
    ws, nb = _gcn_ws(C, Cout, T, V, x)
    _lib.check(_L().agcn_gcn_aggregate_project_fwd_ex(_lib.ptr(x), _lib.ptr(adj), _lib.ptr(wcat), _lib.ptr(bias),
                                                      _lib.ptr(y), _lib.ptr(stats), ws.data_ptr(), nb, N, C, Cout, T, V,
                                                      _lib.ptr(x_amax), _lib.stream()),
               "agcn_gcn_aggregate_project_fwd")
    return y, stats


def aggregate_project_bwd_data(dy, adj, wcat, x_shape, out=None, accumulate=False, add1=None, mask1=None,
                               add2=None, mask2=None, dtp=None, wab=None, dy_amax=None, dtp_amax=None):
    N, C, T, V = x_shape
    Cout = wcat.shape[0]
    dx = out if out is not None else _empty(x_shape, dy)
    ws, nb = _gcn_ws(C, Cout, T, V, dy)
    kinds = {m.dtype for m in (mask1, mask2) if m is not None}
    if len(kinds) > 1:
        raise RuntimeError("agcn_amd: mask1 and mask2 must be of one kind (fp32 tensors or int32 sign bit masks)")
    mbits = int(torch.int32 in kinds)
    mp = _lib.ptr_bits if mbits else _lib.ptr
    if dtp is not None:
        K2 = dtp.shape[1]
        _lib.check(_L().agcn_gcn_aggregate_project_bwd_data_ex(
            _lib.ptr(dy), _lib.ptr(adj), _lib.ptr(wcat), _lib.ptr(dtp), _lib.ptr(wab.reshape(K2, C)), K2, _lib.ptr(dx),
            int(accumulate), _lib.ptr(add1), mp(mask1), _lib.ptr(add2), mp(mask2), mbits, ws.data_ptr(), nb, N, C, Cout,
            T, V, _lib.ptr(dy_amax), _lib.ptr(dtp_amax), _lib.stream()), "agcn_gcn_aggregate_project_bwd_data_fused")
        return dx
    _lib.check(_L().agcn_gcn_aggregate_project_bwd_data_ex(
        _lib.ptr(dy), _lib.ptr(adj), _lib.ptr(wcat), None, None, 0, _lib.ptr(dx), int(accumulate), _lib.ptr(add1),
        mp(mask1), _lib.ptr(add2), mp(mask2), mbits, ws.data_ptr(), nb, N, C, Cout, T, V, _lib.ptr(dy_amax), None,
        _lib.stream()), "agcn_gcn_aggregate_project_bwd_data")
    return dx


def fused_bwd_data_supported(C, Cout, V):
    return bool(_L().agcn_gcn_bwd_data_fused_supported(int(C), int(Cout), int(V)))


def project_bwd_weight(dy, x, adj, Cout, dy_amax=None, x_amax=None):
    N, C, T, V = x.shape
    nbytes = _L().agcn_gcn_project_bwd_weight_workspace(N, C, Cout, T, V)
    ws = torch.empty((nbytes + 3) // 4, dtype=torch.float32, device=x.device)
    dw = _empty((Cout, 3 * C), x)
    _lib.check(_L().agcn_gcn_project_bwd_weight_ex(_lib.ptr(dy), _lib.ptr(x), _lib.ptr(adj), _lib.ptr(dw), _lib.ptr(ws),
                                                   nbytes, N, C, Cout, T, V, _lib.ptr(dy_amax), _lib.ptr(x_amax),
                                                   _lib.stream()),
               "agcn_gcn_project_bwd_weight")
    return dw


def adjacency_bwd(dy, wcat, x, tp, P, alpha=None, wab=None, bab=None, dy_amax=None, x_amax=None):
    N, C, T, V = x.shape
    Cout = wcat.shape[0]
    Ci = (tp.shape[1] if tp is not None else wab.shape[0]) // 6
    nslots = _L().agcn_dadj_num_slots(C, V, T)
    dpart = _empty((N, 3, nslots, V, V), x)
    ws, nb = _gcn_ws(C, Cout, T, V, x)
    _lib.check(_L().agcn_gcn_dadj_ex(_lib.ptr(dy), _lib.ptr(wcat), _lib.ptr(x), _lib.ptr(dpart), ws.data_ptr(), nb, N, C,
                                     Cout, T, V, _lib.ptr(dy_amax), _lib.ptr(x_amax), _lib.stream()), "agcn_gcn_dadj")
    dadj = _empty((N, 3, V, V), x)
    dS = _empty((N, 3, V, V), x)
    dPA = _empty((3, V, V), x)
    dal_part = _empty((N * 3,), x) if alpha is not None else None
    _lib.check(_L().agcn_adjacency_bwd_softmax(_lib.ptr(dpart), _lib.ptr(P), _lib.ptr(alpha), _lib.ptr(dadj),
                                               _lib.ptr(dS), _lib.ptr(dPA), _lib.ptr(dal_part), N, Ci, T, V, nslots,
                                               _lib.stream()), "agcn_adjacency_bwd_softmax")
    nt = _L().agcn_scores_num_tiles(V, T)
    dtp = _empty((N, 6 * Ci, T, V), x)
    dbpart = _empty((N * nt, 6 * Ci), x)
    dbab = _empty((6 * Ci,), x)
    scratch = _scratch(6 * Ci, x)
    dtp_amax = None
    if tp is None:
        nb = _L().agcn_adjacency_fused_workspace(C, Ci)
        ws = _ws(nb, x)
        _lib.check(_L().agcn_adjacency_fused_bwd_scores(
            _lib.ptr(x), _lib.ptr(wab.reshape(6 * Ci, C)), _lib.ptr(bab), _lib.ptr(dS), _lib.ptr(dtp), _lib.ptr(dbpart),
            scratch.data_ptr(), _lib.ptr(dbab), ws.data_ptr(), nb, N, C, Ci, T, V, _lib.stream()),
            "agcn_adjacency_fused_bwd_scores")
    else:
        dtp_amax = _empty((1,), x) if fused_amax_enabled() else None
        _lib.check(_L().agcn_adjacency_bwd_scores_ex(_lib.ptr(tp), _lib.ptr(dS), _lib.ptr(dtp), _lib.ptr(dbpart),
                                                     scratch.data_ptr(), _lib.ptr(dbab), _lib.ptr(dtp_amax), N, Ci, T, V,
                                                     _lib.stream()),
                   "agcn_adjacency_bwd_scores")
    dalpha = dal_part.sum() if dal_part is not None else None
    return dPA, dtp, dbab, dalpha, dadj, dtp_amax


def stc_row_reduce(y, g=None, wv=None, wt=None, want_t=False, want_v=False, scale_t=1.0, scale_v=1.0):
    N, C, T, V = y.shape
    out_t = _empty((N, C, T), y) if want_t else None
    out_v = _empty((N, C, V), y) if want_v else None
    per_row = int(wt is not None and wt.dim() == 3)
    _lib.check(_L().agcn_stc_row_reduce(_lib.ptr(y), _lib.ptr(g), _lib.ptr(wv), _lib.ptr(wt), per_row, _lib.ptr(out_t),
                                        _lib.ptr(out_v), float(scale_t), float(scale_v), N, C, T, V, _lib.stream()),
               "agcn_stc_row_reduce")
    return out_t, out_v


def linear_fwd(x, w, b, act=0):
    N, K = x.shape
    O = w.shape[0]
    out = _empty((N, O), x)
    _lib.check(_L().agcn_linear_fwd(_lib.ptr(x), _lib.ptr(w), _lib.ptr(b), _lib.ptr(out), N, K, O, int(act),
                                    _lib.stream()), "agcn_linear_fwd")
    return out


def linear_bwd(dout, out, x, w, act=0, need_din=True):
    N, K = x.shape
    O = w.shape[0]
    dpre = _empty((N, O), x)
    din = _empty((N, K), x) if need_din else None
    dw, db = _empty((O, K), x), _empty((O,), x)
    _lib.check(_L().agcn_linear_bwd(_lib.ptr(dout), _lib.ptr(out), _lib.ptr(x), _lib.ptr(w), _lib.ptr(dpre),
                                    _lib.ptr(din), _lib.ptr(dw), _lib.ptr(db), N, K, O, int(act), _lib.stream()),
               "agcn_linear_bwd")
    return din, dw, db


def gate_conv_fwd(x, w, b):
    N, C, L = x.shape
    Ks = w.shape[-1]
    a = _empty((N, L), x)
    _lib.check(_L().agcn_gate_conv_fwd(_lib.ptr(x), _lib.ptr(w.reshape(C, Ks)), _lib.ptr(b), _lib.ptr(a), N, C, L, Ks,
                                       _lib.stream()), "agcn_gate_conv_fwd")
    return a


def gate_conv_bwd(da, a, x, w):
    N, C, L = x.shape
    Ks = w.shape[-1]
    dpre = _empty((N, L), x)
    dx, dw, db = _empty((N, C, L), x), _empty((1, C, Ks), x), _empty((1,), x)
    _lib.check(_L().agcn_gate_conv_bwd(_lib.ptr(da), _lib.ptr(a), _lib.ptr(x), _lib.ptr(w.reshape(C, Ks)),
                                       _lib.ptr(dpre), _lib.ptr(dx), _lib.ptr(dw), _lib.ptr(db), N, C, L, Ks,
                                       _lib.stream()), "agcn_gate_conv_bwd")
    return dx, dw, db


class DataBNFunction(torch.autograd.Function):

    @staticmethod
    def forward(ctx, x, w, b, rm, rv, training, sync=None):
        x = x.contiguous()
        N, C, T, V, M = x.shape
        CH = C * V * M
        L = _L()
        if training:
            part = _empty((N, 2, CH), x)
            _lib.check(L.agcn_data_bn_stats(_lib.ptr(x), _lib.ptr(part), N, C, T, V, M, _lib.stream()),
                       "agcn_data_bn_stats")
            (st,), gcount = _bn_coeffs(True, [part], N * T, [(w, b, rm, rv)], sync, N)
        else:
            (st,), gcount = _bn_coeffs(False, [None], N * T, [(w, b, rm, rv)], None, N)
        out = _empty((N * M, C, T, V), x)
        _lib.check(L.agcn_data_bn_apply(_lib.ptr(x), _lib.ptr(st.scale), _lib.ptr(st.shift), _lib.ptr(out), N, C, T, V, M,
                                        _lib.stream()), "agcn_data_bn_apply")
        ctx.st, ctx.sync, ctx.gcount, ctx.training = st, sync, gcount, training
        ctx.save_for_backward(x, w)
        return out

    @staticmethod
    def backward(ctx, dy):
        x, w = ctx.saved_tensors
        st, sync = ctx.st, ctx.sync
        dy = dy.contiguous()
        N, C, T, V, M = x.shape
        CH = C * V * M
        L = _L()
        if not ctx.training:
            dx = dgamma = dbeta = None
            if ctx.needs_input_grad[0]:
                dx = torch.empty_like(x)
                zero = torch.zeros(2 * CH, dtype=torch.float32, device=x.device)
                _lib.check(L.agcn_data_bn_bwd_apply(_lib.ptr(dy), _lib.ptr(x), _lib.ptr(w), _lib.ptr(st.mean),
                                                    _lib.ptr(st.invstd), _lib.ptr(zero), float(ctx.gcount), _lib.ptr(dx),
                                                    N, C, T, V, M, _lib.stream()), "agcn_data_bn_bwd_apply")
            if ctx.needs_input_grad[1] or ctx.needs_input_grad[2]:
                part = _empty((N, 2, CH), x)
                _lib.check(L.agcn_data_bn_bwd_reduce(_lib.ptr(dy), _lib.ptr(x), _lib.ptr(st.mean), _lib.ptr(st.invstd),
                                                     _lib.ptr(part), N, C, T, V, M, _lib.stream()),
                           "agcn_data_bn_bwd_reduce")
                sums = _colsum(part, N, 2 * CH)
                dbeta, dgamma = sums[:CH], sums[CH:]
            return dx, dgamma, dbeta, None, None, None, None
        part = _empty((N, 2, CH), x)
        _lib.check(L.agcn_data_bn_bwd_reduce(_lib.ptr(dy), _lib.ptr(x), _lib.ptr(st.mean), _lib.ptr(st.invstd),
                                             _lib.ptr(part), N, C, T, V, M, _lib.stream()), "agcn_data_bn_bwd_reduce")
        sums = _colsum(part, N, 2 * CH)
        scale = 1.0
        if sync is not None:
            sums = _allreduce_sum(sums, sync)
            scale = 1.0 / sync.world
        dx = None
        if ctx.needs_input_grad[0]:
            dx = torch.empty_like(x)
            _lib.check(L.agcn_data_bn_bwd_apply(_lib.ptr(dy), _lib.ptr(x), _lib.ptr(w), _lib.ptr(st.mean),
                                                _lib.ptr(st.invstd), _lib.ptr(sums), float(ctx.gcount), _lib.ptr(dx), N, C,
                                                T, V, M, _lib.stream()), "agcn_data_bn_bwd_apply")
        dbeta, dgamma = sums[:CH], sums[CH:]
        if scale != 1.0:
            dbeta, dgamma = dbeta * scale, dgamma * scale
        return dx, dgamma, dbeta, None, None, None, None


def data_bn_supported(bn):
    return type(bn) in (torch.nn.BatchNorm1d, torch.nn.SyncBatchNorm)


class PoolFCFunction(torch.autograd.Function):

    @staticmethod
    def forward(ctx, x, w, b, M):
        x = x.contiguous()
        NM, C, T, V = x.shape
        N = NM // M
        rowmean, pooled = _empty((NM, C), x), _empty((N, C), x)
        _lib.check(_L().agcn_pool_fwd(_lib.ptr(x), _lib.ptr(rowmean), _lib.ptr(pooled), N, M, C, T * V, _lib.stream()),
                   "agcn_pool_fwd")
        logits = linear_fwd(pooled, w, b, 0)
        ctx.save_for_backward(pooled, logits, w)
        ctx.shape, ctx.M = (NM, C, T, V), M
        return logits

    @staticmethod
    def backward(ctx, dlogits):
        pooled, logits, w = ctx.saved_tensors
        NM, C, T, V = ctx.shape
        M = ctx.M
        dpooled, dw, db = linear_bwd(dlogits.contiguous(), logits, pooled, w, 0, need_din=True)
        dx = None
        if ctx.needs_input_grad[0]:
            dx = _empty((NM, C, T, V), pooled)
            _lib.check(_L().agcn_pool_bwd(_lib.ptr(dpooled), _lib.ptr(dx), NM // M, M, C, T * V, _lib.stream()),
                       "agcn_pool_bwd")
        return dx, dw, db, None


class STCAttentionFunction(torch.autograd.Function):

    @staticmethod
    def _gates(m_s, mv1, sa_w, sa_b, ta_w, ta_b, f1w, f1b, f2w, f2b, a_s=None):
        if a_s is None:
            a_s = gate_conv_fwd(m_s, sa_w, sa_b)
        if mv1 is None:
            return a_s, None, None, None, None
        a_t = gate_conv_fwd(mv1, ta_w, ta_b)
        m_c = (mv1 * a_t.unsqueeze(1)).mean(-1)
        h = linear_fwd(m_c, f1w, f1b, 1)
        a_c = linear_fwd(h, f2w, f2b, 2)
        return a_s, a_t, a_c, m_c, h

    @staticmethod
    def forward(ctx, y, sa_w, sa_b, ta_w, ta_b, f1w, f1b, f2w, f2b):
        y = y.contiguous()
        N, C, T, V = y.shape
        par = (sa_w, sa_b, ta_w, ta_b, f1w, f1b, f2w, f2b)
        _, m_s = stc_row_reduce(y, want_v=True, scale_v=1.0 / T)
        a_s = STCAttentionFunction._gates(m_s, None, *par)[0]
        mv1, _ = stc_row_reduce(y, wv=a_s, want_t=True, scale_t=1.0 / V)
        _, a_t, a_c, m_c, h = STCAttentionFunction._gates(m_s, mv1, *par, a_s=a_s)
        out = torch.empty_like(y)
        o_amax = _empty((1,), y) if fused_amax_enabled() else None
        INFER_STATS['stc_apply'] += 1
        _lib.check(_L().agcn_stc_apply_ex(_lib.ptr(y), _lib.ptr(a_s), _lib.ptr(a_t), _lib.ptr(a_c), _lib.ptr(out),
                                          _lib.ptr(o_amax), N, C, T, V, _lib.stream()), "agcn_stc_apply")
        _note_out_amax(out, o_amax)
        ctx.save_for_backward(y, m_s, mv1, a_s, a_t, a_c, m_c, h, *par)
        return out

    @staticmethod
    def backward(ctx, dout):
        y, m_s, mv1, a_s, a_t, a_c, m_c, h, *par = ctx.saved_tensors
        sa_w, sa_b, ta_w, ta_b, f1w, f1b, f2w, f2b = par
        dout = dout.contiguous()
        N, C, T, V = y.shape
        P1, P2 = stc_row_reduce(y, g=dout, wv=a_s, wt=a_t, want_t=True, want_v=True)
        da_c = (P1 * a_t.unsqueeze(1)).sum(-1).contiguous()
        da_t = (P1 * a_c.unsqueeze(-1)).sum(1)
        da_s = (P2 * a_c.unsqueeze(-1)).sum(1)
        dh, df2w, df2b = linear_bwd(da_c, a_c, h, f2w, 2)
        dm_c, df1w, df1b = linear_bwd(dh, h, m_c, f1w, 1)
        da_t = (da_t + (dm_c.unsqueeze(-1) * mv1).sum(1) / T).contiguous()
        dmv1 = dm_c.unsqueeze(-1) * a_t.unsqueeze(1) / T
        dmv1_t, dta_w, dta_b = gate_conv_bwd(da_t, a_t, mv1, ta_w)
        dmv1 = ((dmv1 + dmv1_t) / V).contiguous()
        _, R = stc_row_reduce(y, wt=dmv1, want_v=True)
        da_s = (da_s + R.sum(1)).contiguous()
        dm_s, dsa_w, dsa_b = gate_conv_bwd(da_s, a_s, m_s, sa_w)
        dms = (dm_s / T).contiguous()
        dy = torch.empty_like(y)
        _lib.check(_L().agcn_stc_bwd_apply(_lib.ptr(dout), _lib.ptr(a_s), _lib.ptr(a_t), _lib.ptr(a_c), _lib.ptr(dmv1),
                                           _lib.ptr(dms), _lib.ptr(dy), N, C, T, V, _lib.stream()),
                   "agcn_stc_bwd_apply")
        return dy, dsa_w, dsa_b, dta_w, dta_b, df1w, df1b, df2w, df2b


class BNState:
    __slots__ = ("mean", "invstd", "scale", "shift", "S", "eval")

    def __init__(self):
        self.S = 1
        self.eval = False


class SyncBN:
    __slots__ = ("world", "group")

    def __init__(self, world, group=None):
        self.world, self.group = int(world), group


def sync_of(bn_module):
    import torch.distributed as dist
    if isinstance(bn_module, torch.nn.SyncBatchNorm) and dist.is_available() and dist.is_initialized():
        world = dist.get_world_size(bn_module.process_group)
        if world > 1:
            return SyncBN(world, bn_module.process_group)
    return None


def _colsum(slab, nslots, width):
    out = _empty((width,), slab)
    scratch = _scratch(width, slab)
    _lib.check(_L().agcn_colsum(_lib.ptr(slab), int(nslots), int(width), scratch.data_ptr(), _lib.ptr(out),
                                _lib.stream()), "agcn_colsum")
    return out


COLLECTIVES = {'bn': 0, 'grad': 0}


def _allreduce_sum(t, sync):
    import torch.distributed as dist
    COLLECTIVES['bn'] += 1
    dist.all_reduce(t, op=dist.ReduceOp.SUM, group=sync.group)
    return t


def sync_stats(stats_parts, count, sync):
    sums = [_colsum(sp, sp.shape[0], sp.shape[1] * sp.shape[2]) for sp in stats_parts]
    buf = torch.cat(sums) if len(sums) > 1 else sums[0]
    _allreduce_sum(buf, sync)
    out, o = [], 0
    for sp in stats_parts:
        w = sp.shape[1] * sp.shape[2]
        out.append(buf[o:o + w].view(1, 2, sp.shape[2]))
        o += w
    return out


def bn_train_coeffs(stats_part, count, gamma, beta, running_mean, running_var, momentum=BN_MOMENTUM, eps=BN_EPS):
    C = gamma.numel()
    st = BNState()
    st.mean, st.invstd = _empty((C,), gamma), _empty((C,), gamma)
    st.scale, st.shift = _empty((C,), gamma), _empty((C,), gamma)
    nslots = stats_part.shape[0]
    scratch = _scratch(2 * C, gamma)
    _lib.check(_L().agcn_bn_stats_finalize(_lib.ptr(stats_part), nslots, C, float(count), _lib.ptr(gamma),
                                           _lib.ptr(beta), _lib.ptr(running_mean), _lib.ptr(running_var),
                                           float(momentum), float(eps), scratch.data_ptr(), _lib.ptr(st.mean),
                                           _lib.ptr(st.invstd),
                                           _lib.ptr(st.scale), _lib.ptr(st.shift), _lib.stream()),
               "agcn_bn_stats_finalize")
    return st


def bn_eval_coeffs(gamma, beta, running_mean, running_var, eps=BN_EPS):
    C = gamma.numel()
    st = BNState()
    st.eval = True
    st.scale, st.shift = _empty((C,), gamma), _empty((C,), gamma)
    st.mean, st.invstd = _empty((C,), gamma), _empty((C,), gamma)
    _lib.check(_L().agcn_bn_eval_coeff_ex(_lib.ptr(gamma), _lib.ptr(beta), _lib.ptr(running_mean),
                                          _lib.ptr(running_var), float(eps), C, _lib.ptr(st.scale), _lib.ptr(st.shift),
                                          _lib.ptr(st.mean), _lib.ptr(st.invstd), _lib.stream()),
               "agcn_bn_eval_coeff_ex")
    return st


def bn_act_fwd(y1, st1, r=None, st2=None, relu=True, want_bits=False, amax_out=None):
    N, C, T, V = y1.shape
    if st1.S > 1:
        N, C = N // st1.S, C * st1.S
    out = torch.empty_like(y1)
    bits = torch.empty((y1.numel() + 31) // 32, dtype=torch.int32, device=y1.device) if want_bits else None
    mode = 0 if r is None else (1 if st2 is None else 2)
    _lib.check(_L().agcn_bn_act_fwd_ex(_lib.ptr(y1), _lib.ptr(st1.scale), _lib.ptr(st1.shift), _lib.ptr(r),
                                       _lib.ptr(st2.scale) if st2 else None, _lib.ptr(st2.shift) if st2 else None,
                                       _lib.ptr(out), _lib.ptr_bits(bits), _lib.ptr(amax_out), N, C, T * V, mode,
                                       int(relu), _lib.stream()),
               "agcn_bn_act_fwd")
    return (out, bits) if want_bits else out


EVAL_BWD_STATS = {'sums': 0, 'nosums': 0}


def bn_bwd_eval(dout, mask, y1, st1, y2=None, st2=None, want_sums=True, amax_out=None):
    N, C, T, V = dout.shape
    two = st2 is not None
    dy1 = torch.empty_like(dout)
    dy2 = torch.empty_like(dout) if two else None
    part = _empty((N * C * 3,), dout) if want_sums else None
    mbits = int(mask is not None and mask.dtype == torch.int32)
    mptr = _lib.ptr_bits(mask) if mbits else _lib.ptr(mask)
    EVAL_BWD_STATS['sums' if want_sums else 'nosums'] += 1
    _lib.check(_L().agcn_bn_bwd_eval(_lib.ptr(dout), mptr, mbits, _lib.ptr(y1) if want_sums else None,
                                     _lib.ptr(st1.scale), _lib.ptr(y2) if (want_sums and two) else None,
                                     _lib.ptr(st2.scale) if two else None, int(want_sums), _lib.ptr(part),
                                     _lib.ptr(dy1), _lib.ptr(dy2), _lib.ptr(amax_out), N, C, T * V, _lib.stream()),
               "agcn_bn_bwd_eval")
    if not want_sums:
        return dy1, None, None, None, dy2, None, None, None
    dg1, db1, dc1 = _empty((C,), dout), _empty((C,), dout), _empty((C,), dout)
    dg2 = db2 = dc2 = None
    if two:
        dg2, db2, dc2 = _empty((C,), dout), _empty((C,), dout), _empty((C,), dout)
    _lib.check(_L().agcn_bn_bwd_eval_finalize(
        _lib.ptr(part), N, C, _lib.ptr(st1.scale), _lib.ptr(st1.mean), _lib.ptr(st1.invstd),
        _lib.ptr(st2.scale) if two else None, _lib.ptr(st2.mean) if two else None,
        _lib.ptr(st2.invstd) if two else None, _lib.ptr(dg1), _lib.ptr(db1), _lib.ptr(dc1), _lib.ptr(dg2),
        _lib.ptr(db2), _lib.ptr(dc2), _lib.stream()), "agcn_bn_bwd_eval_finalize")
    return dy1, dg1, db1, dc1, dy2, dg2, db2, dc2


def bn_bwd(dout, mask, y1, gamma1, st1, y2=None, gamma2=None, st2=None, sync=None, gcount=None, amax_out=None,
           want_sums=True, bias_out=None):
    if st1.eval:
        dy1, dg1, db1, dc1, dy2, dg2, db2, dc2 = bn_bwd_eval(dout, mask, y1, st1, y2, st2 if y2 is not None else None,
                                                             want_sums, amax_out)
        if bias_out is not None:
            bias_out[:] = [dc1, dc2]
        return dy1, dg1, db1, dy2, dg2, db2
    N, C, T, V = y1.shape
    S = st1.S
    if S > 1:
        N, C = N // S, C * S
        gamma1 = gamma1.repeat(S)
        gamma2 = gamma2.repeat(S) if gamma2 is not None else None
    part = _empty((N * C * 3,), y1)
    coef = _empty((6 * C,), y1)
    dy1 = torch.empty_like(y1)
    dg1, db1 = _empty((C,), y1), _empty((C,), y1)
    dy2 = dg2 = db2 = None
    if y2 is not None:
        dy2 = torch.empty_like(y2)
        dg2, db2 = _empty((C,), y1), _empty((C,), y1)
    mbits = int(mask is not None and mask.dtype == torch.int32)
    mptr = _lib.ptr_bits(mask) if mbits else _lib.ptr(mask)
    if sync is None and amax_out is not None:
        _lib.check(_L().agcn_bn_bwd_reduce(_lib.ptr(dout), mptr, mbits, _lib.ptr(y1), _lib.ptr(y2),
                                           _lib.ptr(part), N, C, T * V, _lib.stream()), "agcn_bn_bwd_reduce")
        _lib.check(_L().agcn_bn_bwd_apply_ex(
            _lib.ptr(part), N, float(N) * float(T * V), 1.0, _lib.ptr(dout), mptr, mbits, _lib.ptr(y1),
            _lib.ptr(gamma1), _lib.ptr(st1.mean), _lib.ptr(st1.invstd), _lib.ptr(y2), _lib.ptr(gamma2),
            _lib.ptr(st2.mean) if st2 else None, _lib.ptr(st2.invstd) if st2 else None, _lib.ptr(coef), _lib.ptr(dy1),
            _lib.ptr(dg1), _lib.ptr(db1), _lib.ptr(dy2), _lib.ptr(dg2), _lib.ptr(db2), _lib.ptr(amax_out), N, C, T * V,
            _lib.stream()), "agcn_bn_bwd_apply")
    elif sync is None:
        _lib.check(_L().agcn_bn_bwd(
            _lib.ptr(dout), mptr, mbits, _lib.ptr(y1), _lib.ptr(gamma1), _lib.ptr(st1.mean), _lib.ptr(st1.invstd),
            _lib.ptr(y2), _lib.ptr(gamma2), _lib.ptr(st2.mean) if st2 else None, _lib.ptr(st2.invstd) if st2 else None,
            _lib.ptr(part), _lib.ptr(coef), _lib.ptr(dy1), _lib.ptr(dg1), _lib.ptr(db1), _lib.ptr(dy2), _lib.ptr(dg2),
            _lib.ptr(db2), N, C, T * V, _lib.stream()), "agcn_bn_bwd")
    else:
        _lib.check(_L().agcn_bn_bwd_reduce(_lib.ptr(dout), mptr, mbits, _lib.ptr(y1), _lib.ptr(y2),
                                           _lib.ptr(part), N, C, T * V, _lib.stream()), "agcn_bn_bwd_reduce")
        sums = _allreduce_sum(_colsum(part, N, 3 * C), sync)
        total = float(gcount) if gcount is not None else float(N * T * V * sync.world)
        _lib.check(_L().agcn_bn_bwd_apply_ex(
            _lib.ptr(sums), 1, total, 1.0 / sync.world, _lib.ptr(dout), mptr, mbits, _lib.ptr(y1),
            _lib.ptr(gamma1), _lib.ptr(st1.mean), _lib.ptr(st1.invstd), _lib.ptr(y2), _lib.ptr(gamma2),
            _lib.ptr(st2.mean) if st2 else None, _lib.ptr(st2.invstd) if st2 else None, _lib.ptr(coef), _lib.ptr(dy1),
            _lib.ptr(dg1), _lib.ptr(db1), _lib.ptr(dy2), _lib.ptr(dg2), _lib.ptr(db2), _lib.ptr(amax_out), N, C, T * V,
            _lib.stream()), "agcn_bn_bwd_apply")
    if S > 1:
        dg1, db1 = dg1.view(S, -1).sum(0), db1.view(S, -1).sum(0)
        if dg2 is not None:
            dg2, db2 = dg2.view(S, -1).sum(0), db2.view(S, -1).sum(0)
    return dy1, dg1, db1, dy2, dg2, db2



class _Ctx:
    pass


def _bn_coeffs(training, stats, count, bns, sync=None, nsamples=None):
    S = bns[0][2].numel() // bns[0][0].numel()
    if not training:
        out = []
        for w, b, rm, rv in bns:
            C = w.numel()
            out.append(bn_eval_coeffs(w, b, rm[:C].contiguous(), rv[:C].contiguous()))
        return out, count
    if S > 1:
        if nsamples is None or nsamples % S:
            raise RuntimeError(f"agcn_amd: GhostBatchNorm with {S} splits needs a batch (x persons) divisible by {S}")
        stats = [_ghost_regroup(sp, S, nsamples) for sp in stats]
        bns = [(w.repeat(S), b.repeat(S), rm, rv) for w, b, rm, rv in bns]
        count = count // S
    if sync is not None:
        stats = sync_stats(stats, count, sync)
        count = count * sync.world
    note_params_changed()
    res = [bn_train_coeffs(sp, count, *bn) for sp, bn in zip(stats, bns)]
    for st in res:
        st.S = S
    return res, count


def _ghost_regroup(stats_part, S, nsamples):
    slots, two, C = stats_part.shape
    nt = slots // nsamples
    return stats_part.view(nsamples // S, S, nt, two, C).permute(0, 2, 3, 1, 4).reshape(nsamples // S * nt, two, S * C)


def gcn_forward(c, x, A, PA, wab, bab, wd, bd, bn, down, training, alpha=None, adaptive=True, sync=None,
                need_bwd=True):
    N, C, T, V = x.shape
    count = N * T * V
    first = down is not None and first_layer_enabled() and bool(_L().agcn_gcn_first_supported(C, wd.shape[0], V))
    x_amax = None if first else _take_out_amax(x)
    if adaptive and adjacency_fused_supported(C, wab.shape[0] // 6, T, V):
        keep = need_bwd and not adjacency_recompute()
        amax_here = None
        if x_amax is None and not first and fused_amax_enabled():
            amax_here = _empty((1,), x)
        if keep:
            P, adj, tp = adjacency_fused_fwd(x, wab, bab, A, PA, alpha, keep_tp=True, x_amax_out=amax_here, x_amax=x_amax)
        else:
            tp = None
            P, adj = adjacency_fused_fwd(x, wab, bab, A, PA, alpha, x_amax_out=amax_here, x_amax=x_amax)
        if amax_here is not None:
            x_amax = amax_here
    elif adaptive:
        tp, _ = conv_fwd(x, wab, bab)
        P, adj = adjacency_fwd(tp, A, PA, alpha)
    else:
        tp = P = None
        adj = A.unsqueeze(0).expand(N, 3, V, V).contiguous()
    if first:
        ypre, st, dpre, st2 = gcn_first_fwd(x, adj, wd, bd, down[0], down[1], want_stats=training)
    else:
        c.g_x_amax = x_amax
        ypre, st = aggregate_project_fwd(x, adj, wd, bd, want_stats=training, x_amax=c.g_x_amax)
    bn2 = None
    if not first:
        dpre = None
    if down is not None:
        if not first:
            dpre, st2 = conv_fwd(x, down[0], down[1], want_stats=training)
        (bn1, bn2), gcount = _bn_coeffs(training, [st, st2], count, [bn, down[2:]], sync, N)
        c.g_amax = _empty((1,), x) if fused_amax_enabled() else None
        out, bits = bn_act_fwd(ypre, bn1, dpre, bn2, relu=True, want_bits=True, amax_out=c.g_amax)
    else:
        (bn1,), gcount = _bn_coeffs(training, [st], count, [bn], sync, N)
        c.g_amax = _empty((1,), x) if fused_amax_enabled() else None
        out, bits = bn_act_fwd(ypre, bn1, x, None, relu=True, want_bits=True, amax_out=c.g_amax)
    c.g_sync, c.g_count = sync, gcount
    c.g_bits = bits
    c.g_x, c.g_tp, c.g_P, c.g_adj, c.g_ypre, c.g_dpre, c.g_out = x, tp, P, adj, ypre, dpre, out
    c.g_bn1, c.g_bn2 = bn1, bn2
    c.g_params = (wab, wd, bn[0], down[0] if down is not None else None, down[2] if down is not None else None)
    c.g_bab = bab
    c.g_alpha, c.g_adaptive = alpha, adaptive
    return out


def gcn_backward(c, dout, extra_add=None, extra_mask=None):
    x, tp, P, adj, ypre, dpre, out = c.g_x, c.g_tp, c.g_P, c.g_adj, c.g_ypre, c.g_dpre, c.g_out
    wab, wd, gamma1, wdown, gamma2 = c.g_params
    Cout = wd.shape[0]
    dy_amax = _empty((1,), dout) if fused_amax_enabled() else None
    c.g_dbias = []
    dypre, dg1, db1, ddpre, dg2, db2 = bn_bwd(dout, c.g_bits, ypre, gamma1, c.g_bn1, dpre, gamma2, c.g_bn2,
                                              sync=c.g_sync, gcount=c.g_count, amax_out=dy_amax,
                                              want_sums=getattr(c, 'g_want_sums', True), bias_out=c.g_dbias)
    x_amax = getattr(c, 'g_x_amax', None)
    dwd = _side_run(lambda: project_bwd_weight(dypre, x, adj, Cout, dy_amax, x_amax), (dypre, x, adj, dy_amax, x_amax))
    dPA = dwab = dbab = dalpha = dtp = dtp_amax = None
    if c.g_adaptive:
        dPA, dtp, dbab, dalpha, _, dtp_amax = adjacency_bwd(dypre, wd, x, tp, P, c.g_alpha, wab, c.g_bab,
                                                            dy_amax=dy_amax, x_amax=x_amax)
        dwab = _side_run(lambda: conv_bwd_weight(dtp, x, wab.shape, 1, dtp_amax, x_amax), (dtp, x, dtp_amax, x_amax))
    fuse = dtp is not None and fused_bwd_data_supported(x.shape[1], Cout, x.shape[3])
    ftp = dict(dtp=dtp, wab=wab) if fuse else {}
    ftp['dy_amax'] = dy_amax
    if fuse:
        ftp['dtp_amax'] = dtp_amax
    if dpre is None:
        dx = aggregate_project_bwd_data(dypre, adj, wd, x.shape, add1=dout, mask1=c.g_bits, add2=extra_add,
                                        mask2=extra_mask, **ftp)
    else:
        dx = aggregate_project_bwd_data(dypre, adj, wd, x.shape, add1=extra_add, mask1=extra_mask, **ftp)
    if dtp is not None and not fuse:
        conv_bwd_data(dtp, wab, x.shape, out=dx, accumulate=True)
    c.g_dalpha = dalpha
    dwdown = None
    if dpre is not None:
        dwdown = _side_run(lambda: conv_bwd_weight(ddpre, x, wdown.shape), (ddpre, x))
        conv_bwd_data(ddpre, wdown, x.shape, out=dx, accumulate=True)
    _side_join()
    return dx, dPA, dwab, dbab, dwd, dg1, db1, dwdown, dg2, db2


def tcn_forward(c, g, w, b, bn, stride, res_x, res, relu, training, sync=None, pad=None):
    N, C, T, V = g.shape
    if res is not None:
        To = conv_out_frames(T, w.shape[2], stride, pad)
        Tr = res_x.shape[2] if isinstance(res, str) else conv_out_frames(res_x.shape[2], 1, stride, 0)
        if Tr != To:
            raise RuntimeError(f"agcn_amd: the residual has {Tr} frames but the temporal convolution ({w.shape[2]} taps, "
                               f"stride {stride}, padding {(w.shape[2] - 1) // 2 if pad is None else pad}) gives {To} "
                               f"for {T} input frames; they must agree (the reference fails here too)")
    g_amax = getattr(c, 'g_amax', None) if getattr(c, 'g_out', None) is g else None
    if g_amax is None and getattr(c, 'g_out', None) is None:
        g_amax = _take_out_amax(g)
    zpre, st = conv_fwd(g, w, b, stride, want_stats=training, x_amax=g_amax, pad=pad)
    To = zpre.shape[2]
    count = N * To * V
    rpre = bn2 = None
    if res is None or isinstance(res, str):
        (bn1,), gcount = _bn_coeffs(training, [st], count, [bn], sync, N)
        o_amax = _empty((1,), g) if fused_amax_enabled() else None
        out, bits = bn_act_fwd(zpre, bn1, None if res is None else res_x, None, relu=relu, want_bits=True,
                               amax_out=o_amax)
    else:
        rpre, st2 = conv_fwd(res_x, res[0], res[1], stride, want_stats=training)
        (bn1, bn2), gcount = _bn_coeffs(training, [st, st2], count, [bn, res[2:]], sync, N)
        o_amax = _empty((1,), g) if fused_amax_enabled() else None
        out, bits = bn_act_fwd(zpre, bn1, rpre, bn2, relu=relu, want_bits=True, amax_out=o_amax)
    _note_out_amax(out, o_amax)
    c.t_sync, c.t_count = sync, gcount
    c.t_bits = bits
    c.t_g, c.t_zpre, c.t_rpre, c.t_out, c.t_bn1, c.t_bn2 = g, zpre, rpre, out, bn1, bn2
    c.t_g_amax = g_amax
    c.t_resx, c.t_res_identity = res_x, isinstance(res, str)
    c.t_params = (w, bn[0], res[0] if isinstance(res, tuple) else None, res[2] if isinstance(res, tuple) else None)
    c.t_stride, c.t_relu, c.t_pad = stride, relu, pad
    return out


def tcn_backward(c, dout, join=True):
    w, gamma1, wres, gamma2 = c.t_params
    mask = c.t_bits if c.t_relu else None
    dz_amax = _empty((1,), dout) if fused_amax_enabled() else None
    c.t_dbias = []
    dzpre, dg1, db1, drpre, dg2, db2 = bn_bwd(dout, mask, c.t_zpre, gamma1, c.t_bn1, c.t_rpre, gamma2, c.t_bn2,
                                              sync=c.t_sync, gcount=c.t_count, amax_out=dz_amax,
                                              want_sums=getattr(c, 't_want_sums', True), bias_out=c.t_dbias)
    t_g, t_stride, t_pad = c.t_g, c.t_stride, getattr(c, 't_pad', None)
    t_g_amax = getattr(c, 't_g_amax', None)
    dw = _side_run(lambda: conv_bwd_weight(dzpre, t_g, w.shape, t_stride, dz_amax, t_g_amax, pad=t_pad),
                   (dzpre, t_g, dz_amax, t_g_amax))
    dg = conv_bwd_data(dzpre, w, c.t_g.shape, c.t_stride, dy_amax=dz_amax, pad=t_pad)
    dwres = None
    if drpre is not None:
        t_resx = c.t_resx
        dwres = _side_run(lambda: conv_bwd_weight(drpre, t_resx, wres.shape, t_stride), (drpre, t_resx))
    if join:
        _side_join()
    return dg, dw, dg1, db1, drpre, dwres, dg2, db2


ERR_UNSUPPORTED = -3

_PARAM_EPOCH = [0]


def note_params_changed():
    _PARAM_EPOCH[0] += 1


def infer_fold_enabled():
    return os.environ.get('AGCN_INFER_FOLD', '1') != '0'


INFER_STATS = {'aagcn_unit_fused': 0, 'tconv_infer': 0, 'stc_apply': 0}


def _fold(bn):
    w, b, rm, rv = bn
    C = w.numel()
    s = w / torch.sqrt(rv[:C] + BN_EPS)
    return s, b - rm[:C] * s


def _fold_conv(w, b, bn):
    s, sh = _fold(bn)
    return (w * s[:, None, None, None]).contiguous(), (b * s + sh).contiguous()


def gcn_unit_infer(x, adj, wcat, bias, res=None, x2=None, w2=None, relu=True):
    N, C, T, V = x.shape
    Cout = wcat.shape[0]
    K2 = 0 if x2 is None else x2.shape[1]
    nbytes = _L().agcn_gcn_unit_infer_workspace(C, Cout, K2, T, V)
    ws = _ws(nbytes, x)
    y = _empty((N, Cout, T, V), x)
    rc = _L().agcn_gcn_unit_infer(_lib.ptr(x), _lib.ptr(adj), _lib.ptr(wcat), _lib.ptr(bias), _lib.ptr(res),
                                  _lib.ptr(x2), _lib.ptr(w2), K2, 1 if relu else 0, _lib.ptr(y), ws.data_ptr(), nbytes,
                                  N, C, Cout, T, V, _lib.stream())
    if rc == ERR_UNSUPPORTED:
        return None
    _lib.check(rc, "agcn_gcn_unit_infer")
    return y


def conv9_infer(x, w, b, res=None, relu=True, stride=1):
    N, Cin, T, V = x.shape
    Cout = w.shape[0]
    To = conv_out_frames(T, 9, stride)
    ws, nbytes = _conv_ws(Cin, Cout, T, V, 9, stride, x)
    y = _empty((N, Cout, To, V), x)
    rc = _L().agcn_conv9_infer(_lib.ptr(x), _lib.ptr(w), _lib.ptr(b), _lib.ptr(res), 1 if relu else 0, _lib.ptr(y),
                               ws.data_ptr(), nbytes, N, Cin, Cout, T, V, stride, _lib.stream())
    if rc == ERR_UNSUPPORTED:
        return None
    _lib.check(rc, "agcn_conv9_infer")
    return y


def tconv_infer(x, w, b, a_s=None, a_t=None, a_c=None, res=None, relu=True, stride=1, pad=None, x_amax=None):
    N, Cin, T, V = x.shape
    Cout, Cin2, taps, one = w.shape
    assert Cin2 == Cin and one == 1
    pad = (taps - 1) // 2 if pad is None else pad
    To = conv_out_frames(T, taps, stride, pad)
    if To < 1:
        raise ValueError(f"agcn_amd: a {taps}-frame kernel with padding {pad} does not fit {T} frames")
    ws, nbytes = _conv_ws(Cin, Cout, T, V, taps, stride, x, pad)
    y = _empty((N, Cout, To, V), x)
    rc = _L().agcn_tconv_infer(_lib.ptr(x), _lib.ptr(w), _lib.ptr(b), _lib.ptr(a_s), _lib.ptr(a_t), _lib.ptr(a_c),
                               _lib.ptr(res), 1 if relu else 0, _lib.ptr(y), ws.data_ptr(), nbytes, N, Cin, Cout, T, V,
                               taps, stride, pad, _lib.ptr(x_amax), _lib.stream())
    if rc == ERR_UNSUPPORTED:
        return None
    _lib.check(rc, "agcn_tconv_infer")
    INFER_STATS['tconv_infer'] += 1
    return y


def _cache_key(srcs):
    return (_PARAM_EPOCH[0],) + tuple((t.data_ptr(), t._version) for t in srcs if t is not None)


def tcn_infer(x, w, b, bn, stride, pad, cache=None):
    key = _cache_key([w, b, *bn])
    f = cache.get('folded') if cache is not None else None
    if f is None or f[0] != key:
        f = (key,) + _fold_conv(w, b, bn)
        if cache is not None:
            cache['folded'] = f
    return tconv_infer(x.contiguous(), f[1], f[2], relu=False, stride=stride, pad=pad)


def aagcn_unit_infer(x, p, cache=None):
    x = x.contiguous()
    N, C, T, V = x.shape
    if C < 32 or _L().agcn_gemm_mode() not in (b'bf16x6', b'bf16'):
        return None
    srcs = [t for wb in p['conv_d'] for t in wb] + [t for q in (p['ab'] or []) for t in q]
    srcs += [*p['gbn'], p['tw'], p['tb'], *p['tbn']] + list(p['down'] or []) + list(p['res'] or [])
    key = _cache_key(srcs)
    f = cache.get('folded') if cache is not None else None
    if f is None or f[0] != key:
        Cout = p['conv_d'][0][0].shape[0]
        wd = torch.cat([w.view(Cout, C) for w, _ in p['conv_d']], dim=1)
        bd = p['conv_d'][0][1] + p['conv_d'][1][1] + p['conv_d'][2][1]
        s1, sh1 = _fold(p['gbn'])
        wdf = (wd * s1[:, None]).contiguous()
        bias = bd * s1 + sh1
        w2 = None
        if p['down'] is not None:
            dw, db = _fold_conv(p['down'][0], p['down'][1], p['down'][2:])
            w2 = dw.reshape(Cout, C)
            bias = bias + db
        twf, tbf = _fold_conv(p['tw'], p['tb'], p['tbn'])
        rwf = rbf = None
        if p['res'] is not None:
            rwf, rbf = _fold_conv(p['res'][0], p['res'][1], p['res'][2:])
        wab = bab = None
        if p['ab'] is not None:
            wab = torch.cat([t for wa, _, wb_, _ in p['ab'] for t in (wa, wb_)], 0).contiguous()
            bab = torch.cat([t for _, ba, _, bb in p['ab'] for t in (ba, bb)], 0).contiguous()
        f = (key, wdf, bias.contiguous(), w2, twf, tbf, rwf, rbf, wab, bab)
        if cache is not None:
            cache['folded'] = f
    _, wdf, bias, w2, twf, tbf, rwf, rbf, wab, bab = f
    if wab is not None and adjacency_fused_supported(C, wab.shape[0] // 6, T, V):
        _, adj = adjacency_fused_fwd(x, wab, bab, None, p['PA'], p['alpha'])
    elif wab is not None:
        tp, _ = conv_fwd(x, wab, bab)
        _, adj = adjacency_fwd(tp, None, p['PA'], p['alpha'])
    else:
        adj = p['A'].unsqueeze(0).expand(N, 3, V, V).contiguous()
    if w2 is None:
        g = gcn_unit_infer(x, adj, wdf, bias, res=x)
    else:
        g = gcn_unit_infer(x, adj, wdf, bias, x2=x, w2=w2)
    if g is None:
        return None
    a_s = a_t = a_c = None
    if p['attn'] is not None:
        _, m_s = stc_row_reduce(g, want_v=True, scale_v=1.0 / T)
        a_s = STCAttentionFunction._gates(m_s, None, *p['attn'])[0]
        mv1, _ = stc_row_reduce(g, wv=a_s, want_t=True, scale_t=1.0 / V)
        _, a_t, a_c, _, _ = STCAttentionFunction._gates(m_s, mv1, *p['attn'], a_s=a_s)
    if p['res_mode'] == 0:
        r = None
    elif p['res_mode'] == 1:
        r = x
    else:
        r, _ = conv_fwd(x, rwf, rbf, p['stride'])
    y = tconv_infer(g, twf, tbf, a_s, a_t, a_c, res=r, relu=True, stride=p['stride'], pad=p['pad'])
    if y is not None:
        INFER_STATS['aagcn_unit_fused'] += 1
    return y


def unit_infer(x, A, PA, wab, bab, wd, bd, gbn, down, tw, tb, tbn, res_mode, res, stride, alpha=None, adaptive=True,
               cache=None):
    x = x.contiguous()
    N, C, T, V = x.shape
    Cout = wd.shape[0]
    if C < 32:
        return None
    srcs = [wd, bd, *gbn, tw, tb, *tbn] + (list(down) if down is not None else []) + \
           (list(res) if isinstance(res, tuple) else [])
    key = (_PARAM_EPOCH[0],) + tuple((t.data_ptr(), t._version) for t in srcs)
    f = cache.get('folded') if cache is not None else None
    if f is None or f[0] != key:
        s1, sh1 = _fold(gbn)
        wdf = (wd * s1[:, None]).contiguous()
        bias = bd * s1 + sh1
        w2 = None
        if down is not None:
            s2, sh2 = _fold(down[2:])
            w2 = (down[0].reshape(Cout, C) * s2[:, None]).contiguous()
            bias = bias + down[1] * s2 + sh2
        s3, sh3 = _fold(tbn)
        twf = (tw * s3[:, None, None, None]).contiguous()
        tbf = tb * s3 + sh3
        rwf = rbf = None
        if isinstance(res, tuple):
            s4, sh4 = _fold(res[2:])
            rwf = (res[0] * s4[:, None, None, None]).contiguous()
            rbf = res[1] * s4 + sh4
        f = (key, wdf, bias.contiguous(), w2, twf, tbf.contiguous(), rwf, rbf)
        if cache is not None:
            cache['folded'] = f
    _, wdf, bias, w2, twf, tbf, rwf, rbf = f
    if adaptive and adjacency_fused_supported(C, wab.shape[0] // 6, T, V):
        _, adj = adjacency_fused_fwd(x, wab, bab, A, PA, alpha)
    elif adaptive:
        tp, _ = conv_fwd(x, wab, bab)
        _, adj = adjacency_fwd(tp, A, PA, alpha)
    else:
        adj = A.unsqueeze(0).expand(N, 3, V, V).contiguous()
    if down is None:
        g = gcn_unit_infer(x, adj, wdf, bias, res=x)
    else:
        g = gcn_unit_infer(x, adj, wdf, bias, x2=x, w2=w2)
    if g is None:
        return None
    if res_mode == 0:
        r = None
    elif res_mode == 1:
        r = x
    else:
        r, _ = conv_fwd(x, rwf, rbf, stride)
    if tw.shape[2] == 9:
        return conv9_infer(g, twf, tbf, r, relu=True, stride=stride)
    return tconv_infer(g, twf, tbf, res=r, relu=True, stride=stride)


def _bias_grad(slot, k, n, like, needed=True):
    if slot and slot[k] is not None:
        return slot[k]
    if slot:
        return None
    return torch.zeros(n, dtype=torch.float32, device=like.device) if needed else None


class UnitGCNFunction(torch.autograd.Function):

    @staticmethod
    def forward(ctx, x, A, PA, wab, bab, wd, bd, bn_w, bn_b, bn_rm, bn_rv, down_w, down_b, dbn_w, dbn_b, dbn_rm,
                dbn_rv, training, alpha=None, adaptive=True, sync=None):
        c = _Ctx()
        down = None if down_w is None else (down_w, down_b, dbn_w, dbn_b, dbn_rm, dbn_rv)
        out = gcn_forward(c, x.contiguous(), A, PA, wab, bab, wd, bd, (bn_w, bn_b, bn_rm, bn_rv), down, training,
                          alpha, adaptive, sync, need_bwd=any(ctx.needs_input_grad))
        ctx.c, ctx.training = c, training
        ctx.has_down = down is not None
        _note_out_amax(out, getattr(c, 'g_amax', None))
        return out

    @staticmethod
    def backward(ctx, dout):
        ng = ctx.needs_input_grad
        ctx.c.g_want_sums = any(ng[i] for i in (6, 7, 8, 12, 13, 14))
        dx, dPA, dwab, dbab, dwd, dg1, db1, dwdown, dg2, db2 = gcn_backward(ctx.c, dout.contiguous())
        dbd = _bias_grad(ctx.c.g_dbias, 0, dwd.shape[0], dout)
        dbdown = _bias_grad(ctx.c.g_dbias, 1, dwd.shape[0], dout, ctx.has_down)
        dalpha = ctx.c.g_dalpha
        if dalpha is not None:
            dalpha = dalpha.reshape(1)
        ctx.c = None
        return (dx, None, dPA, dwab, dbab, dwd, dbd, dg1, db1, None, None, dwdown, dbdown, dg2, db2, None, None, None,
                dalpha, None, None)


class UnitTCNFunction(torch.autograd.Function):

    @staticmethod
    def forward(ctx, x, w, b, bn_w, bn_b, bn_rm, bn_rv, stride, training, sync=None, pad=None):
        c = _Ctx()
        out = tcn_forward(c, x.contiguous(), w, b, (bn_w, bn_b, bn_rm, bn_rv), stride, None, None, False, training,
                          sync, pad)
        ctx.c, ctx.training = c, training
        return out

    @staticmethod
    def backward(ctx, dout):
        ctx.c.t_want_sums = any(ctx.needs_input_grad[i] for i in (2, 3, 4))
        dg, dw, dg1, db1, _, _, _, _ = tcn_backward(ctx.c, dout.contiguous())
        dbias = _bias_grad(ctx.c.t_dbias, 0, dw.shape[0], dout)
        ctx.c = None
        return dg, dw, dbias, dg1, db1, None, None, None, None, None, None


class TCNResidualFunction(torch.autograd.Function):

    @staticmethod
    def forward(ctx, g, x, w, b, bn_w, bn_b, bn_rm, bn_rv, res_mode, rw, rb, rbn_w, rbn_b, rbn_rm, rbn_rv, stride,
                training, sync=None, pad=None):
        c = _Ctx()
        res = None if res_mode == 0 else ('identity' if res_mode == 1 else (rw, rb, rbn_w, rbn_b, rbn_rm, rbn_rv))
        x = x.contiguous() if x is not None else None
        out = tcn_forward(c, g.contiguous(), w, b, (bn_w, bn_b, bn_rm, bn_rv), stride, x, res, True, training, sync,
                          pad)
        ctx.c, ctx.training, ctx.res_mode, ctx.stride = c, training, res_mode, stride
        ctx.x_shape = tuple(x.shape) if x is not None else None
        return out

    @staticmethod
    def backward(ctx, dout):
        c = ctx.c
        dout = dout.contiguous()
        c.t_want_sums = any(ctx.needs_input_grad[i] for i in (3, 4, 5, 10, 11, 12))
        dg, dw, dg1, db1, drpre, dwres, dg2, db2 = tcn_backward(c, dout)
        dtb = _bias_grad(c.t_dbias, 0, dw.shape[0], dout)
        drb = _bias_grad(c.t_dbias, 1, dw.shape[0], dout, ctx.res_mode == 2)
        dx = None
        if ctx.res_mode == 1:
            dx = torch.where(c.t_out > 0, dout, torch.zeros_like(dout))
        elif ctx.res_mode == 2:
            dx = conv_bwd_data(drpre, c.t_params[2], ctx.x_shape, ctx.stride)
        ctx.c = None
        return (dg, dx, dw, dtb, dg1, db1, None, None, None,
                dwres, drb, dg2, db2, None, None, None, None, None, None)


class TCNGCNUnitFunction(torch.autograd.Function):

    @staticmethod
    def forward(ctx, x, A, PA, wab, bab, wd, bd, gbn_w, gbn_b, gbn_rm, gbn_rv, down_w, down_b, dbn_w, dbn_b, dbn_rm,
                dbn_rv, tw, tb, tbn_w, tbn_b, tbn_rm, tbn_rv, res_mode, rw, rb, rbn_w, rbn_b, rbn_rm, rbn_rv, stride,
                training, sync=None):
        c = _Ctx()
        x = x.contiguous()
        down = None if down_w is None else (down_w, down_b, dbn_w, dbn_b, dbn_rm, dbn_rv)
        g = gcn_forward(c, x, A, PA, wab, bab, wd, bd, (gbn_w, gbn_b, gbn_rm, gbn_rv), down, training, sync=sync,
                        need_bwd=any(ctx.needs_input_grad))
        res = None if res_mode == 0 else ('identity' if res_mode == 1 else (rw, rb, rbn_w, rbn_b, rbn_rm, rbn_rv))
        out = tcn_forward(c, g, tw, tb, (tbn_w, tbn_b, tbn_rm, tbn_rv), stride, x, res, True, training, sync)
        ctx.c, ctx.training, ctx.has_down, ctx.res_mode, ctx.stride = c, training, down is not None, res_mode, stride
        return out

    @staticmethod
    def backward(ctx, dout):
        c = ctx.c
        dout = dout.contiguous()
        ng = ctx.needs_input_grad
        c.g_want_sums = any(ng[i] for i in (6, 7, 8, 12, 13, 14))
        c.t_want_sums = any(ng[i] for i in (18, 19, 20, 25, 26, 27))
        _SIDE_SCOPE[0] += 1
        try:
            dg, dtw, dtg, dtb, drpre, drw, drg, drb = tcn_backward(c, dout, join=False)
            if ctx.res_mode == 1:
                gres = gcn_backward(c, dg, extra_add=dout, extra_mask=c.t_bits)
            else:
                gres = gcn_backward(c, dg)
        finally:
            _SIDE_SCOPE[0] -= 1
        dx, dPA, dwab, dbab, dwd, dg1, db1, dwdown, dg2, db2 = gres
        if ctx.res_mode == 2:
            conv_bwd_data(drpre, c.t_params[2], c.g_x.shape, ctx.stride, out=dx, accumulate=True)
        Cout = dwd.shape[0]
        dbd = _bias_grad(c.g_dbias, 0, Cout, dout)
        dbdown = _bias_grad(c.g_dbias, 1, Cout, dout, ctx.has_down)
        dtbias = _bias_grad(c.t_dbias, 0, Cout, dout)
        drbias = _bias_grad(c.t_dbias, 1, Cout, dout, ctx.res_mode == 2)
        ctx.c = None
        return (dx, None, dPA, dwab, dbab, dwd, dbd, dg1, db1, None, None,
                dwdown, dbdown, dg2, db2, None, None,
                dtw, dtbias, dtg, dtb, None, None, None,
                drw, drbias, drg, drb, None, None, None, None, None)
```

### include/agcn_hip.h

```cpp
#ifndef AGCN_HIP_H
#define AGCN_HIP_H

#include <stddef.h>

#ifdef __cplusplus
extern "C" {
#endif

#define AGCN_OK 0
#define AGCN_ERR_ARG (-1)
#define AGCN_ERR_WORKSPACE (-2)
#define AGCN_ERR_UNSUPPORTED (-3)

int agcn_version(void);
const char* agcn_arch(void);

const char* agcn_last_kernel(void);
const char* agcn_gemm_mode(void);
const char* agcn_chain_mode(void);

int agcn_conv_tile_frames(int V, int T_out);
int agcn_conv_num_tiles(int V, int T_out);
int agcn_conv_stats_tiles(int Cin, int Cout, int T_out, int V, int taps, int stride);
int agcn_scores_num_tiles(int V, int T);
int agcn_dadj_num_slots(int C, int V, int T);

size_t agcn_conv_workspace(int Cin, int Cout, int T, int V, int taps, int stride);
int agcn_conv_fwd(const float* x, const float* w, const float* bias, float* y, float* stats_part, void* workspace,
                  size_t workspace_bytes, int N, int Cin, int Cout, int T, int V, int taps, int stride, void* stream);
int agcn_conv_bwd_data(const float* dy, const float* w, float* dx, int accumulate, const float* add1,
                       const float* mask1, const float* add2, const float* mask2, void* workspace,
                       size_t workspace_bytes, int N, int Cin, int Cout, int T, int V, int taps, int stride,
                       void* stream);
size_t agcn_conv_bwd_weight_workspace(int N, int Cin, int Cout, int T, int V, int taps, int stride);
int agcn_conv_bwd_weight(const float* dy, const float* x, float* dw, void* workspace, size_t workspace_bytes, int N,
                         int Cin, int Cout, int T, int V, int taps, int stride, void* stream);

size_t agcn_gcn_workspace(int C, int Cout, int T, int V);
int agcn_gcn_stats_tiles(int C, int Cout, int T, int V);
int agcn_gcn_stats_slots(int N, int C, int Cout, int T, int V);
int agcn_gcn_aggregate_project_fwd(const float* x, const float* adj, const float* wcat, const float* bias, float* y,
                                   float* stats_part, void* workspace, size_t workspace_bytes, int N, int C, int Cout,
                                   int T, int V, void* stream);
int agcn_bn_act_fwd_ex(const float* y1, const float* scale1, const float* shift1, const float* r, const float* scale2,
                       const float* shift2, float* out, unsigned* sign_bits, float* absmax_out, int N, int C, int P,
                       int res_mode, int relu, void* stream);
int agcn_bn_bwd_apply_ex(const float* part, int nrows, double count, float param_grad_scale, const float* dout,
                         const void* mask, int mask_bits, const float* y1, const float* gamma1, const float* mean1,
                         const float* invstd1, const float* y2, const float* gamma2, const float* mean2,
                         const float* invstd2, float* coef, float* dy1, float* dgamma1, float* dbeta1, float* dy2,
                         float* dgamma2, float* dbeta2, float* absmax1_out, int N, int C, int P, void* stream);
int agcn_gcn_aggregate_project_fwd_ex(const float* x, const float* adj, const float* wcat, const float* bias, float* y,
                                      float* stats_part, void* workspace, size_t workspace_bytes, int N, int C, int Cout,
                                      int T, int V, const float* x_absmax, void* stream);
int agcn_gcn_aggregate_project_bwd_data_ex(const float* dy, const float* adj, const float* wcat, const float* dtp,
                                           const float* w2, int K2, float* dx, int accumulate, const float* add1,
                                           const float* mask1, const float* add2, const float* mask2, int mask_bits,
                                           void* workspace, size_t workspace_bytes, int N, int C, int Cout, int T, int V,
                                           const float* dy_absmax, const float* dtp_absmax, void* stream);
int agcn_gcn_dadj_ex(const float* dy, const float* wcat, const float* x, float* dadj_part, void* workspace,
                     size_t workspace_bytes, int N, int C, int Cout, int T, int V, const float* dy_absmax,
                     const float* x_absmax, void* stream);
int agcn_adjacency_bwd_scores_ex(const float* tp, const float* dS, float* dtp, float* dbpart, void* scratch, float* db,
                                 float* dtp_absmax_out, int N, int Ci, int T, int V, void* stream);
int agcn_conv_bwd_weight_ex(const float* dy, const float* x, float* dw, void* workspace, size_t workspace_bytes, int N,
                            int Cin, int Cout, int T, int V, int taps, int stride, const float* dy_absmax,
                            const float* x_absmax, void* stream);
int agcn_gcn_project_bwd_weight_ex(const float* dy, const float* x, const float* adj, float* dwcat, void* workspace,
                                   size_t workspace_bytes, int N, int C, int Cout, int T, int V, const float* dy_absmax,
                                   const float* x_absmax, void* stream);
int agcn_absmax(const float* x, long n, float* out, void* stream);
int agcn_conv_fwd_ex(const float* x, const float* w, const float* bias, float* y, float* stats_part, void* workspace,
                     size_t workspace_bytes, int N, int Cin, int Cout, int T, int V, int taps, int stride,
                     const float* x_absmax, void* stream);
int agcn_conv_bwd_data_ex(const float* dy, const float* w, float* dx, int accumulate, const float* add1,
                          const float* mask1, const float* add2, const float* mask2, void* workspace,
                          size_t workspace_bytes, int N, int Cin, int Cout, int T, int V, int taps, int stride,
                          const float* dy_absmax, void* stream);

size_t agcn_tconv_workspace(int Cin, int Cout, int T, int V, int taps, int stride, int pad);
int agcn_tconv_stats_tiles(int Cin, int Cout, int T_out, int V, int taps, int stride, int pad);
int agcn_tconv_fwd(const float* x, const float* w, const float* bias, float* y, float* stats_part, void* workspace,
                   size_t workspace_bytes, int N, int Cin, int Cout, int T, int V, int taps, int stride, int pad,
                   const float* x_absmax, void* stream);
int agcn_tconv_bwd_data(const float* dy, const float* w, float* dx, int accumulate, const float* add1,
                        const float* mask1, const float* add2, const float* mask2, void* workspace,
                        size_t workspace_bytes, int N, int Cin, int Cout, int T, int V, int taps, int stride, int pad,
                        const float* dy_absmax, void* stream);
size_t agcn_tconv_bwd_weight_workspace(int N, int Cin, int Cout, int T, int V, int taps, int stride, int pad);
int agcn_tconv_bwd_weight(const float* dy, const float* x, float* dw, void* workspace, size_t workspace_bytes, int N,
                          int Cin, int Cout, int T, int V, int taps, int stride, int pad, const float* dy_absmax,
                          const float* x_absmax, void* stream);

int agcn_gcn_first_supported(int C, int Cout, int V);
int agcn_gcn_first_tiles(int T, int V);
int agcn_gcn_first_fwd(const float* x, const float* adj, const float* wcat, const float* bias, const float* wdown,
                       const float* bdown, float* ypre, float* ystats, float* dpre, float* dstats, int N, int C, int Cout,
                       int T, int V, void* stream);

size_t agcn_gcn_unit_infer_workspace(int C, int Cout, int K2, int T, int V);
int agcn_gcn_unit_infer(const float* x, const float* adj, const float* wcat, const float* bias, const float* res,
                        const float* x2, const float* w2, int K2, int relu, float* y, void* workspace,
                        size_t workspace_bytes, int N, int C, int Cout, int T, int V, void* stream);
int agcn_conv9_infer(const float* x, const float* w, const float* bias, const float* res, int relu, float* y,
                     void* workspace, size_t workspace_bytes, int N, int Cin, int Cout, int T, int V, int stride,
                     void* stream);

int agcn_tconv_infer(const float* x, const float* w, const float* bias, const float* a_s, const float* a_t,
                     const float* a_c, const float* res, int relu, float* y, void* workspace, size_t workspace_bytes,
                     int N, int Cin, int Cout, int T, int V, int taps, int stride, int pad, const float* x_absmax,
                     void* stream);

int agcn_gcn_aggregate_project_bwd_data(const float* dy, const float* adj, const float* wcat, float* dx,
                                        int accumulate, const float* add1, const float* mask1, const float* add2,
                                        const float* mask2, int mask_bits, void* workspace, size_t workspace_bytes, int N, int C,
                                        int Cout, int T, int V, void* stream);
int agcn_gcn_bwd_data_fused_supported(int C, int Cout, int V);
int agcn_gcn_aggregate_project_bwd_data_fused(const float* dy, const float* adj, const float* wcat, const float* dtp,
                                              const float* w2, int K2, float* dx, int accumulate, const float* add1,
                                              const float* mask1, const float* add2, const float* mask2, int mask_bits,
                                              void* workspace, size_t workspace_bytes, int N, int C, int Cout, int T,
                                              int V, void* stream);
size_t agcn_gcn_project_bwd_weight_workspace(int N, int C, int Cout, int T, int V);
int agcn_gcn_project_bwd_weight(const float* dy, const float* x, const float* adj, float* dwcat, void* workspace,
                                size_t workspace_bytes, int N, int C, int Cout, int T, int V, void* stream);
int agcn_gcn_dadj(const float* dy, const float* wcat, const float* x, float* dadj_part, void* workspace,
                  size_t workspace_bytes, int N, int C, int Cout, int T, int V, void* stream);

int agcn_adjacency_fwd(const float* tp, const float* A, const float* PA, const float* alpha, float* spart, float* P,
                       float* adj, int N, int Ci, int T, int V, void* stream);
int agcn_adjacency_fused_supported(int C, int Ci, int T, int V);
size_t agcn_adjacency_fused_workspace(int C, int Ci);
int agcn_adjacency_fused_fwd(const float* x, const float* wab, const float* bab, const float* A, const float* PA,
                             const float* alpha, float* tp_out, float* spart, float* P, float* adj, void* workspace,
                             size_t workspace_bytes, int N, int C, int Ci, int T, int V, void* stream);
int agcn_adjacency_fused_fwd_ex(const float* x, const float* wab, const float* bab, const float* A, const float* PA,
                                const float* alpha, float* tp_out, float* spart, float* P, float* adj, float* x_absmax_out,
                                const float* x_absmax_in, void* workspace, size_t workspace_bytes, int N, int C, int Ci, int T,
                                int V, void* stream);
int agcn_adjacency_fused_bwd_scores(const float* x, const float* wab, const float* bab, const float* dS, float* dtp,
                                    float* dbpart, void* scratch, float* db, void* workspace, size_t workspace_bytes,
                                    int N, int C, int Ci, int T, int V, void* stream);
int agcn_adjacency_bwd_softmax(const float* dadj_part, const float* P, const float* alpha, float* dadj, float* dS,
                               float* dPA, float* dalpha_part, int N, int Ci, int T, int V, int nslots, void* stream);
int agcn_adjacency_bwd_scores(const float* tp, const float* dS, float* dtp, float* dbpart, void* scratch, float* db,
                              int N, int Ci, int T, int V, void* stream);

size_t agcn_colsum_scratch_bytes(int W);
int agcn_colsum(const float* X, int nslots, int W, void* scratch, float* out, void* stream);
int agcn_bn_stats_finalize(const float* stats_part, int nslots, int C, double count, const float* gamma,
                           const float* beta, float* running_mean, float* running_var, float momentum, float eps,
                           void* scratch , float* mean, float* invstd,
                           float* scale, float* shift, void* stream);
int agcn_bn_eval_coeff(const float* gamma, const float* beta, const float* running_mean, const float* running_var,
                       float eps, int C, float* scale, float* shift, void* stream);
int agcn_bn_act_fwd(const float* y1, const float* scale1, const float* shift1, const float* r, const float* scale2,
                    const float* shift2, float* out, unsigned* sign_bits, int N, int C, int P, int res_mode, int relu,
                    void* stream);
int agcn_bn_bwd_reduce(const float* dout, const void* mask, int mask_bits, const float* y1, const float* y2, float* part,
                       int N, int C, int P, void* stream);
int agcn_bn_bwd_apply(const float* part, int nrows, double count, float param_grad_scale, const float* dout,
                      const void* mask, int mask_bits, const float* y1, const float* gamma1, const float* mean1,
                      const float* invstd1, const float* y2, const float* gamma2, const float* mean2, const float* invstd2, float* coef,
                      float* dy1, float* dgamma1, float* dbeta1, float* dy2, float* dgamma2, float* dbeta2, int N, int C,
                      int P, void* stream);
int agcn_bn_bwd(const float* dout, const void* mask, int mask_bits, const float* y1, const float* gamma1,
                const float* mean1, const float* invstd1, const float* y2, const float* gamma2, const float* mean2, const float* invstd2,
                float* part, float* coef, float* dy1, float* dgamma1, float* dbeta1, float* dy2, float* dgamma2,
                float* dbeta2, int N, int C, int P, void* stream);
int agcn_bn_eval_coeff_ex(const float* gamma, const float* beta, const float* running_mean, const float* running_var,
                          float eps, int C, float* scale, float* shift, float* mean, float* invstd, void* stream);
int agcn_bn_bwd_eval(const float* dout, const void* mask, int mask_bits, const float* y1, const float* scale1,
                     const float* y2, const float* scale2, int want_sums, float* part , float* dy1,
                     float* dy2, float* absmax1_out, int N, int C, int P, void* stream);
int agcn_bn_bwd_eval_finalize(const float* part, int nrows, int C, const float* scale1, const float* mean1,
                              const float* invstd1, const float* scale2, const float* mean2, const float* invstd2,
                              float* dgamma1, float* dbeta1, float* dbias1, float* dgamma2, float* dbeta2,
                              float* dbias2, void* stream);

int agcn_stc_row_reduce(const float* y, const float* g, const float* wv, const float* wt, int wt_per_row, float* out_t,
                        float* out_v, float scale_t, float scale_v, int N, int C, int T, int V, void* stream);
int agcn_stc_apply(const float* y, const float* a_s, const float* a_t, const float* a_c, float* out, int N, int C, int T,
                   int V, void* stream);
int agcn_stc_apply_ex(const float* y, const float* a_s, const float* a_t, const float* a_c, float* out, float* absmax_out,
                      int N, int C, int T, int V, void* stream);
int agcn_stc_bwd_apply(const float* dout, const float* a_s, const float* a_t, const float* a_c, const float* dmv,
                       const float* dms, float* dy, int N, int C, int T, int V, void* stream);

int agcn_data_bn_stats(const float* x, float* part, int N, int C, int T, int V, int M, void* stream);
int agcn_data_bn_apply(const float* x, const float* scale, const float* shift, float* out, int N, int C, int T, int V,
                       int M, void* stream);
int agcn_data_bn_bwd_reduce(const float* dy, const float* x, const float* mean, const float* invstd, float* part, int N,
                            int C, int T, int V, int M, void* stream);
int agcn_data_bn_bwd_apply(const float* dy, const float* x, const float* gamma, const float* mean, const float* invstd,
                           const float* sums, double count, float* dx, int N, int C, int T, int V, int M, void* stream);
int agcn_pool_fwd(const float* x, float* rowmean, float* pooled, int N, int M, int C, int P, void* stream);
int agcn_pool_bwd(const float* dpooled, float* dx, int N, int M, int C, int P, void* stream);
int agcn_linear_fwd(const float* in, const float* w, const float* b, float* out, int N, int K, int O, int act,
                    void* stream);
int agcn_linear_bwd(const float* dout, const float* out, const float* in, const float* w, float* dpre, float* din,
                    float* dw, float* db, int N, int K, int O, int act, void* stream);
int agcn_gate_conv_fwd(const float* in, const float* w, const float* b, float* a, int N, int C, int L, int Ks,
                       void* stream);
int agcn_gate_conv_bwd(const float* da, const float* a, const float* in, const float* w, float* dpre, float* din,
                       float* dw, float* db, int N, int C, int L, int Ks, void* stream);

size_t agcn_sgd_step_workspace(long n);
int agcn_sgd_step(float* param, const float* grad, float* momentum_buf, long n, float lr, float momentum,
                  float weight_decay, int nesterov, float max_norm, float grad_scale, int first_step, void* workspace,
                  size_t workspace_bytes, float* norm_out, void* stream);

#ifdef __cplusplus
}
#endif
#endif
```

Measured before the change: 1053 clips/s.

## Fuse BN backward partial sums into temporal conv backward-data epilogue

Adds a BNS variant of the bf16/f16x3 conv GEMM and producer-consumer kernels whose epilogue, while writing dx, also computes per-channel partial sums of masked dz, dz*y1 and dz*y2 for the following batch-norm backward. The Python side passes these partials to the BN backward apply step, skipping the separate bn_bwd_reduce pass over the activation tensor. This trades an extra full read of dout/y1/y2 for extra loads and reductions inside the conv epilogue, which adds register pressure and partial-sum writes. It is enabled by default through an environment flag and only applies to the f16x3 path with S==1 and non-eval BN.

```diff
diff --git a/2s-agcn_amd/csrc/conv_gemm_bf16.hip b/2s-agcn_amd/csrc/conv_gemm_bf16.hip
--- a/2s-agcn_amd/csrc/conv_gemm_bf16.hip
+++ b/2s-agcn_amd/csrc/conv_gemm_bf16.hip
@@ -41,8 +41,15 @@
   GateArgs gate;
   int off_gate;
 };
-template <bool GATE> struct BfArgsOf { typedef BfArgs type; };
-template <> struct BfArgsOf<true> { typedef GateBfArgs type; };
+struct BnBfArgs : BfArgs {
+  const float* bn_y1;
+  const float* bn_y2;
+  const unsigned* bn_bits;
+  float* bn_part;
+};
+template <bool GATE, bool BNS = false> struct BfArgsOf { typedef BfArgs type; };
+template <> struct BfArgsOf<true, false> { typedef GateBfArgs type; };
+template <> struct BfArgsOf<false, true> { typedef BnBfArgs type; };
 
 struct BfPackArgs {
   const float* w;
@@ -103,8 +110,8 @@
   }
 }
 
-template <int TAPS, int NPL, int WQ, int TM, int TN = 1, bool F16 = false, bool GATE = false>
-__global__ void __launch_bounds__(NT, (TAPS == 1 && TM == 2 && TN == 1) ? 4 : 2) conv_gemm_bf16_kernel(const typename BfArgsOf<GATE>::type a) {
+template <int TAPS, int NPL, int WQ, int TM, int TN = 1, bool F16 = false, bool GATE = false, bool BNS = false>
+__global__ void __launch_bounds__(NT, (TAPS == 1 && TM == 2 && TN == 1) ? 4 : 2) conv_gemm_bf16_kernel(const typename BfArgsOf<GATE, BNS>::type a) {
   constexpr int BM = TM * 32;
   constexpr int A_PLANE = TAPS * 2 * BM * 16;
   constexpr int A4 = NPL * A_PLANE / 16;
@@ -311,14 +318,15 @@
   EpiPtrs ep;
   ep.out = a.out; ep.add1 = a.add1; ep.mask1 = a.mask1; ep.add2 = a.add2; ep.mask2 = a.mask2; ep.stats = a.stats;
   ep.accumulate = a.accumulate; ep.relu = a.relu;
+  if constexpr (BNS) { ep.bn_y1 = a.bn_y1; ep.bn_y2 = a.bn_y2; ep.bn_bits = a.bn_bits; ep.bn_part = a.bn_part; }
   const long Pfull = (long)a.T_full * V;
   const long rows0 = (long)n * a.M * Pfull + ((long)t0 * a.out_fs + a.out_fo) * V;
-  epilogue_rows<BM, NW, 4 * TN>(ep, tile, TP, bias_s, red, a.M, m0, rows0, Pfull, nvalid, poff, (long)n * a.ntiles + tile_id);
-}
-
-
-template <int TAPS, int NPL, int R, int NWP = 4, bool F16 = false, bool GATE = false>
-__global__ void __launch_bounds__((8 + NWP) * 64, 3) conv_pc_kernel(const typename BfArgsOf<GATE>::type a) {
+  epilogue_rows<BM, NW, 4 * TN, BNS>(ep, tile, TP, bias_s, red, a.M, m0, rows0, Pfull, nvalid, poff, (long)n * a.ntiles + tile_id);
+}
+
+
+template <int TAPS, int NPL, int R, int NWP = 4, bool F16 = false, bool GATE = false, bool BNS = false>
+__global__ void __launch_bounds__((8 + NWP) * 64, 3) conv_pc_kernel(const typename BfArgsOf<GATE, BNS>::type a) {
   constexpr int TM = 4, BM = 128, NWC = 8, NTALL = (NWC + NWP) * 64, NTP = NWP * 64;
   constexpr int SLOT = NPL * 2 * BM * 16;
   constexpr int PIECES = SLOT / 1024;
@@ -573,9 +581,10 @@
   EpiPtrs ep;
   ep.out = a.out; ep.add1 = a.add1; ep.mask1 = a.mask1; ep.add2 = a.add2; ep.mask2 = a.mask2; ep.stats = a.stats;
   ep.accumulate = a.accumulate; ep.relu = a.relu;
+  if constexpr (BNS) { ep.bn_y1 = a.bn_y1; ep.bn_y2 = a.bn_y2; ep.bn_bits = a.bn_bits; ep.bn_part = a.bn_part; }
   const long Pfull = (long)a.T_full * V;
   const long rows0 = (long)n * a.M * Pfull + ((long)t0 * a.out_fs + a.out_fo) * V;
-  epilogue_rows<BM, NWC, 4>(ep, tile, TP, bias_s, red, a.M, m0, rows0, Pfull, nvalid, poff, (long)n * a.ntiles + tile_id);
+  epilogue_rows<BM, NWC, 4, BNS>(ep, tile, TP, bias_s, red, a.M, m0, rows0, Pfull, nvalid, poff, (long)n * a.ntiles + tile_id);
 }
 
 template <int TAPS, int BM, int NPL, bool F16 = false>
@@ -644,15 +653,20 @@
   void* ws;
   size_t ws_bytes;
   int stats_tiles;
+  const float* bn_y1;
+  const float* bn_y2;
+  const unsigned* bn_bits;
+  float* bn_part;
 };
 
 inline size_t gate_bytes(const BfGeom& g) { return 4 * (size_t)gate_lds_floats(g.FW, g.nchunks * CK); }
 
-template <int TAPS, int NPL, int WQ, int TM, int TN = 1, bool F16 = false, bool GATE = false>
+template <int TAPS, int NPL, int WQ, int TM, int TN = 1, bool F16 = false, bool GATE = false, bool BNS = false>
 int launch_bf(BfProblem& p, hipStream_t stream) {
   constexpr int BM = TM * 32;
-  typename BfArgsOf<GATE>::type a;
+  typename BfArgsOf<GATE, BNS>::type a;
   static_cast<BfArgs&>(a) = p.a;
+  if constexpr (BNS) { a.bn_y1 = p.bn_y1; a.bn_y2 = p.bn_y2; a.bn_bits = p.bn_bits; a.bn_part = p.bn_part; }
   BfGeom g = bf_geometry<TAPS, BM, TN>(a.V, a.T_out, a.src_stride, a.M, a.Kinner);
   if constexpr (GATE) {
     a.gate = p.gate;
@@ -677,10 +691,11 @@
     int rc = agcn_check_launch();
     if (rc) return rc;
   }
-  auto kern = conv_gemm_bf16_kernel<TAPS, NPL, WQ, TM, TN, F16, GATE>;
+  auto kern = conv_gemm_bf16_kernel<TAPS, NPL, WQ, TM, TN, F16, GATE, BNS>;
   static unsigned char lds_ok[AGCN_MAX_DEVICES] = {};
   if (int e = agcn_allow_big_lds_rt(reinterpret_cast<const void*>(kern), lds_ok)) return e;
   if (GATE) AGCN_NOTE_KERNEL("conv_gemm_bf16_kernel<%d, %d, %d, %d, %d, %s, true> [gates on load]", TAPS, NPL, WQ, TM, TN, F16 ? "true" : "false");
+  else if (BNS) AGCN_NOTE_KERNEL("conv_gemm_bf16_kernel<%d, %d, %d, %d, %d, %s, false, true> [bn-bwd sums]", TAPS, NPL, WQ, TM, TN, F16 ? "true" : "false");
   else AGCN_NOTE_KERNEL("conv_gemm_bf16_kernel<%d, %d, %d, %d, %d, %s>", TAPS, NPL, WQ, TM, TN, F16 ? "true" : "false");
   hipLaunchKernelGGL(kern, dim3((unsigned)(a.N * g.ntiles * g.nmb)), dim3(NT), g.smem_bytes, stream, a);
   return agcn_check_launch();
@@ -718,11 +733,12 @@
   return v == 1;
 }
 
-template <int TAPS, int NPL, int R = 5, int NWP = 4, bool F16 = false, bool GATE = false>
+template <int TAPS, int NPL, int R = 5, int NWP = 4, bool F16 = false, bool GATE = false, bool BNS = false>
 int launch_pc(BfProblem& p, hipStream_t stream) {
   constexpr int BM = 128;
-  typename BfArgsOf<GATE>::type a;
+  typename BfArgsOf<GATE, BNS>::type a;
   static_cast<BfArgs&>(a) = p.a;
+  if constexpr (BNS) { a.bn_y1 = p.bn_y1; a.bn_y2 = p.bn_y2; a.bn_bits = p.bn_bits; a.bn_part = p.bn_part; }
   BfGeom g = bf_geometry_pc<TAPS, NPL, R>(a.V, a.T_out, a.M, a.Kinner);
   if constexpr (GATE) {
     a.gate = p.gate;
@@ -742,12 +758,13 @@
   hipLaunchKernelGGL((pack_weights_slots_kernel<TAPS, BM, NPL, F16>), dim3(g.nmb * g.nchunks * TAPS), dim3(256), 0, stream, pk);
   int rc = agcn_check_launch();
   if (rc) return rc;
-  auto kern = conv_pc_kernel<TAPS, NPL, R, NWP, F16, GATE>;
+  auto kern = conv_pc_kernel<TAPS, NPL, R, NWP, F16, GATE, BNS>;
   static unsigned char lds_ok[AGCN_MAX_DEVICES] = {};
   if (int e = agcn_allow_big_lds_rt(reinterpret_cast<const void*>(kern), lds_ok)) return e;
   static const int dbg = getenv("AGCN_CB_DBG") ? atoi(getenv("AGCN_CB_DBG")) : 0;
   a.dbg = dbg;
   if (GATE) AGCN_NOTE_KERNEL("conv_pc_kernel<%d, %d, %d, %d, %s, true> [gates on load]", TAPS, NPL, R, NWP, F16 ? "true" : "false");
+  else if (BNS) AGCN_NOTE_KERNEL("conv_pc_kernel<%d, %d, %d, %d, %s, false, true> [bn-bwd sums]", TAPS, NPL, R, NWP, F16 ? "true" : "false");
   else AGCN_NOTE_KERNEL("conv_pc_kernel<%d, %d, %d, %d, %s>", TAPS, NPL, R, NWP, F16 ? "true" : "false");
   hipLaunchKernelGGL(kern, dim3((unsigned)(a.N * g.ntiles * g.nmb)), dim3((8 + NWP) * 64), g.smem_bytes, stream, a);
   return agcn_check_launch();
@@ -761,14 +778,18 @@
   return g.smem_bytes + (gate ? gate_bytes(g) : 0) <= 160 * 1024 && g.FW * p.a.V <= 512;
 }
 
+static inline bool conv_nwp2() {
+  static const int nwp2 = getenv("AGCN_CONV_NWP2") ? atoi(getenv("AGCN_CONV_NWP2")) : 0;
+  return nwp2 != 0;
+}
+
 template <int TAPS, int WQ, bool GATE = false>
 int launch_npl(BfProblem& p, int npl, hipStream_t s) {
   const BfGeom g128 = bf_geometry<TAPS, 128>(p.a.V, p.a.T_out, p.a.src_stride, p.a.M, p.a.Kinner);
   const bool fits128 = g128.smem_bytes + (GATE ? gate_bytes(g128) : 0) <= 160 * 1024;
   if constexpr (TAPS >= 3) {
     if (pc_applies<TAPS>(p, npl, GATE)) {
-      static const int nwp2 = getenv("AGCN_CONV_NWP2") ? atoi(getenv("AGCN_CONV_NWP2")) : 0;
-      if (nwp2 && !GATE) return launch_pc<TAPS, 3, 5, 2>(p, s);
+      if (conv_nwp2() && !GATE) return launch_pc<TAPS, 3, 5, 2>(p, s);
       if (p.fwd_f16) return launch_pc<TAPS, 2, 5, 4, true, GATE>(p, s);
       return launch_pc<TAPS, 3, 5, 4, false, GATE>(p, s);
     }
@@ -793,6 +814,62 @@
   }
   if (npl == 1) return launch_bf<TAPS, 1, WQ, 2, 1, false, GATE>(p, s);
   return npl == 2 ? launch_bf<TAPS, 2, WQ, 2, 1, false, GATE>(p, s) : launch_bf<TAPS, 3, WQ, 2, 1, false, GATE>(p, s);
+}
+
+template <int TAPS, int WQ>
+int bns_variant(const BfProblem& p, int npl, int* ntiles) {
+  static_assert(TAPS >= 3, "the f16x3 temporal kernels");
+  if (!p.fwd_f16 || npl != 3 || p.a.T_out <= 0) return 0;
+  if (pc_applies<TAPS>(p, npl)) {
+    if (conv_nwp2()) return 0;
+    *ntiles = bf_geometry_pc<TAPS, 2, 5>(p.a.V, p.a.T_out, p.a.M, p.a.Kinner).ntiles;
+    return 1;
+  }
+  const BfGeom g128 = bf_geometry<TAPS, 128>(p.a.V, p.a.T_out, p.a.src_stride, p.a.M, p.a.Kinner);
+  if (p.a.M % 128 == 0 && g128.smem_bytes <= 160 * 1024) return 0;
+  if (agcn_bf16_conv_wide(TAPS, p.a.M)) {
+    const BfGeom g = bf_geometry<TAPS, 64, 2>(p.a.V, p.a.T_out, p.a.src_stride, p.a.M, p.a.Kinner);
+    if (g.smem_bytes <= 160 * 1024 && (g.FW * p.a.V + 3) / 4 <= 3 * 64) {
+      *ntiles = g.ntiles;
+      return 2;
+    }
+  }
+  const BfGeom g = bf_geometry<TAPS, 64, 1>(p.a.V, p.a.T_out, p.a.src_stride, p.a.M, p.a.Kinner);
+  if (g.smem_bytes > 160 * 1024 || (g.FW * p.a.V + 3) / 4 > WQ * 64) return 0;
+  *ntiles = g.ntiles;
+  return 3;
+}
+
+template <int TAPS, int WQ>
+int launch_bns(BfProblem& p, int variant, hipStream_t s) {
+  switch (variant) {
+    case 1: return launch_pc<TAPS, 2, 5, 4, true, false, true>(p, s);
+    case 2: return launch_bf<TAPS, 2, 3, 2, 2, true, false, true>(p, s);
+    case 3: return launch_bf<TAPS, 2, WQ, 2, 1, true, false, true>(p, s);
+    default: return AGCN_ERR_UNSUPPORTED;
+  }
+}
+
+int bns_variant_rt(int taps, const BfProblem& p, int npl, int* ntiles) {
+  switch (taps) {
+    case 3: return bns_variant<3, 2>(p, npl, ntiles);
+    case 4: return bns_variant<4, 2>(p, npl, ntiles);
+    case 5: return bns_variant<5, 2>(p, npl, ntiles);
+    case 7: return bns_variant<7, 2>(p, npl, ntiles);
+    case 9: return bns_variant<9, 2>(p, npl, ntiles);
+    default: return 0;
+  }
+}
+
+int launch_bns_rt(int taps, BfProblem& p, int variant, hipStream_t s) {
+  switch (taps) {
+    case 3: return launch_bns<3, 2>(p, variant, s);
+    case 4: return launch_bns<4, 2>(p, variant, s);
+    case 5: return launch_bns<5, 2>(p, variant, s);
+    case 7: return launch_bns<7, 2>(p, variant, s);
+    case 9: return launch_bns<9, 2>(p, variant, s);
+    default: return AGCN_ERR_UNSUPPORTED;
+  }
 }
 
 }
@@ -1048,3 +1125,94 @@
   t = bf_geometry<1, 128>(V, T, 1, Cin, Cout).pack_bytes; if (t > b) b = t;
   return b + 256;
 }
+
+namespace {
+
+struct BnsPlan {
+  int nlaunch, rows;
+  int taps[2], variant[2], ntiles[2];
+};
+
+void bns_problem(BfProblem& p, int i, int Cin, int Cout, int T, int V, int taps, int stride, int pad) {
+  BfArgs& a = p.a;
+  a.M = Cin; a.Kinner = Cout; a.in_rows = Cout; a.V = V;
+  a.T_src = (T + 2 * pad - taps) / stride + 1; a.T_full = T; a.src_stride = 1;
+  p.sa_m = taps; p.sa_c = (long)Cin * taps;
+  if (stride == 1) {
+    a.T_out = T; a.out_fs = 1; a.out_fo = 0; a.f_off = pad - (taps - 1);
+    p.tap_mul = 1; p.tap_add = 0; p.tap_flip_from = taps - 1;
+  } else if (i == 0) {
+    a.T_out = (T + 1) / 2; a.out_fs = 2; a.out_fo = 0; a.f_off = -2;
+    p.tap_mul = 2; p.tap_add = 0; p.tap_flip_from = 8;
+  } else {
+    a.T_out = T / 2; a.out_fs = 2; a.out_fo = 1; a.f_off = -1;
+    p.tap_mul = 2; p.tap_add = 1; p.tap_flip_from = 8;
+  }
+}
+
+bool bns_plan(BnsPlan& pl, int Cin, int Cout, int T, int V, int taps, int stride, int pad) {
+  pl.nlaunch = pl.rows = 0;
+  const int npl = agcn_gemm_precision();
+  if (npl != 3 || !bf16_fwd_f16x3(npl)) return false;
+  if (Cin <= 0 || Cout <= 0 || T <= 0 || V <= 0 || V > 32) return false;
+  const bool nine = taps == 9 && pad == 4 && (stride == 1 || stride == 2);
+  const bool odd = (taps == 3 || taps == 5 || taps == 7) && stride == 1 && pad >= 0 && pad <= (taps - 1) / 2 &&
+                   T + 2 * pad >= taps;
+  if (!nine && !odd) return false;
+  const int n = (stride == 2 && T / 2 > 0) ? 2 : 1;
+  for (int i = 0; i < n; ++i) {
+    BfProblem p = {};
+    p.fwd_f16 = 1;
+    bns_problem(p, i, Cin, Cout, T, V, taps, stride, pad);
+    pl.taps[i] = stride == 1 ? taps : (i == 0 ? 5 : 4);
+    pl.variant[i] = bns_variant_rt(pl.taps[i], p, npl, &pl.ntiles[i]);
+    if (!pl.variant[i]) return false;
+    pl.rows += pl.ntiles[i];
+  }
+  pl.nlaunch = n;
+  return true;
+}
+
+}
+
+extern "C" {
+
+int agcn_tconv_bwd_data_bn_rows(int Cin, int Cout, int T, int V, int taps, int stride, int pad) {
+  BnsPlan pl;
+  return bns_plan(pl, Cin, Cout, T, V, taps, stride, pad) ? pl.rows : 0;
+}
+
+int agcn_tconv_bwd_data_bn(const float* dy, const float* w, float* dx, int accumulate, const float* add1,
+                           const float* mask1, const float* add2, const float* mask2, void* workspace,
+                           size_t workspace_bytes, int N, int Cin, int Cout, int T, int V, int taps, int stride, int pad,
+                           const float* dy_absmax, const float* bn_y1, const float* bn_y2, const void* bn_bits,
+                           float* bn_part, int bn_rows, void* stream) {
+  if (!dy || !w || !dx || !workspace || !bn_y1 || !bn_bits || !bn_part || N <= 0 || Cin <= 0 || Cout <= 0 || T <= 0 ||
+      V <= 0 || V > 32)
+    return AGCN_ERR_ARG;
+  BnsPlan pl;
+  if (!bns_plan(pl, Cin, Cout, T, V, taps, stride, pad)) return AGCN_ERR_UNSUPPORTED;
+  if ((long)N * pl.rows != (long)bn_rows) return AGCN_ERR_ARG;
+  hipStream_t s = (hipStream_t)stream;
+  BfProblem p = {};
+  BfArgs& a = p.a;
+  p.fwd_f16 = 1;
+  p.ws = workspace; p.ws_bytes = workspace_bytes;
+  const int To = (T + 2 * pad - taps) / stride + 1;
+  if (int rc = bf16_in_absmax(p, dy_absmax, dy, (long)N * Cout * To * V, s)) return rc;
+  a.in = dy; a.out = dx; a.accumulate = accumulate;
+  a.add1 = add1; a.mask1 = mask1; a.add2 = add2; a.mask2 = mask2;
+  a.N = N;
+  p.w = w;
+  p.bn_y1 = bn_y1; p.bn_y2 = bn_y2; p.bn_bits = static_cast<const unsigned*>(bn_bits);
+  long row0 = 0;
+  for (int i = 0; i < pl.nlaunch; ++i) {
+    bns_problem(p, i, Cin, Cout, T, V, taps, stride, pad);
+    p.bn_part = bn_part + row0 * Cin * 3;
+    if (int rc = launch_bns_rt(pl.taps[i], p, pl.variant[i], s)) return rc;
+    row0 += (long)N * pl.ntiles[i];
+  }
+  return 0;
+}
+
+}
diff --git a/2s-agcn_amd/csrc/epilogue.h b/2s-agcn_amd/csrc/epilogue.h
--- a/2s-agcn_amd/csrc/epilogue.h
+++ b/2s-agcn_amd/csrc/epilogue.h
@@ -10,9 +10,13 @@
   float* stats;
   int accumulate;
   int relu;
+  const float* bn_y1 = nullptr;
+  const float* bn_y2 = nullptr;
+  const unsigned* bn_bits = nullptr;
+  float* bn_part = nullptr;
 };
 
-template <int BM, int NW, int XB>
+template <int BM, int NW, int XB, bool BNS = false>
 __device__ __forceinline__ void epilogue_rows(const EpiPtrs& e, const float* tile, int TP, const float* bias_s,
                                               float* red, int M, int m0, long rows0, long P, int nvalid,
                                               const int (&poff)[XB], long stats_slot) {
@@ -21,13 +25,14 @@
   const int wave = __builtin_amdgcn_readfirstlane(tid >> 6);
   constexpr int RG = (XB >= 8) ? 1 : ((XB >= 4) ? 2 : 4), NG = BM / (NW * RG);
   static_assert(BM % (NW * RG) == 0, "row groups must tile the block");
-  const bool has_extra = e.accumulate || e.add1 || e.add2;
-  float ex[2][5][RG][XB];
+  const bool has_extra = BNS || e.accumulate || e.add1 || e.add2;
+  constexpr int NF = BNS ? 8 : 5;
+  float ex[2][NF][RG][XB];
   auto row_base = [&](int k, int g) __attribute__((always_inline)) {
     const int m = min(m0 + (k * NW + wave) * RG + g, M - 1);
     return rows0 + (long)m * P;
   };
-  auto load_extras = [&](int k, float (&x)[5][RG][XB]) __attribute__((always_inline)) {
+  auto load_extras = [&](int k, float (&x)[NF][RG][XB]) __attribute__((always_inline)) {
 #pragma unroll
     for (int g = 0; g < RG; ++g) {
       const long base = row_base(k, g);
@@ -40,6 +45,11 @@
         if (e.mask1) x[2][g][u] = e.mask1[idx];
         if (e.add2) x[3][g][u] = e.add2[idx];
         if (e.mask2) x[4][g][u] = e.mask2[idx];
+        if constexpr (BNS) {
+          x[5][g][u] = e.bn_y1[idx];
+          if (e.bn_y2) x[6][g][u] = e.bn_y2[idx];
+          x[7][g][u] = __builtin_bit_cast(float, e.bn_bits[idx >> 5]);
+        }
       }
     }
   };
@@ -78,6 +88,7 @@
       if (m >= M) break;
       const long base = row_base(k, g);
       const float bval = bias_s[r0 + g];
+      float s0 = 0.f, s1 = 0.f, s2 = 0.f;
 #pragma unroll
       for (int u = 0; u < XB; ++u) {
         const int q = lane + 64 * u;
@@ -87,6 +98,22 @@
         if (e.add2) v += (!e.mask2 || ex[k & 1][4][g][u] > 0.f) ? ex[k & 1][3][g][u] : 0.f;
         if (e.relu) v = fmaxf(v, 0.f);
         if (q < nvalid) e.out[base + poff[u]] = v;
+        if constexpr (BNS) {
+          const unsigned word = __builtin_bit_cast(unsigned, ex[k & 1][7][g][u]);
+          const bool pass = q < nvalid && ((word >> ((base + poff[u]) & 31)) & 1u) != 0u;
+          const float dz = pass ? v : 0.f;
+          s0 += dz;
+          s1 += dz * ex[k & 1][5][g][u];
+          if (e.bn_y2) s2 += dz * ex[k & 1][6][g][u];
+        }
+      }
+      if constexpr (BNS) {
+        s0 = half_sum(s0); s1 = half_sum(s1); s2 = half_sum(s2);
+        s0 += __shfl_xor(s0, 32); s1 += __shfl_xor(s1, 32); s2 += __shfl_xor(s2, 32);
+        if (lane == 0) {
+          float* dst = e.bn_part + (stats_slot * M + m) * 3;
+          dst[0] = s0; dst[1] = s1; dst[2] = s2;
+        }
       }
     }
   }
diff --git a/2s-agcn_amd/lib.py b/2s-agcn_amd/lib.py
--- a/2s-agcn_amd/lib.py
+++ b/2s-agcn_amd/lib.py
@@ -43,6 +43,8 @@
     "agcn_tconv_stats_tiles": (_I, [_I] * 7),
     "agcn_tconv_fwd": (_I, [_P] * 6 + [_Z] + [_I] * 8 + [_P, _P]),
     "agcn_tconv_bwd_data": (_I, [_P, _P, _P, _I, _P, _P, _P, _P, _P, _Z] + [_I] * 8 + [_P, _P]),
+    "agcn_tconv_bwd_data_bn_rows": (_I, [_I] * 7),
+    "agcn_tconv_bwd_data_bn": (_I, [_P, _P, _P, _I, _P, _P, _P, _P, _P, _Z] + [_I] * 8 + [_P] * 5 + [_I, _P]),
     "agcn_tconv_bwd_weight_workspace": (_Z, [_I] * 8),
     "agcn_tconv_bwd_weight": (_I, [_P] * 4 + [_Z] + [_I] * 8 + [_P] * 3),
     "agcn_bn_act_fwd_ex": (_I, [_P, _P, _P, _P, _P, _P, _P, _P, _P, _I, _I, _I, _I, _I, _P]),
diff --git a/2s-agcn_amd/ops.py b/2s-agcn_amd/ops.py
--- a/2s-agcn_amd/ops.py
+++ b/2s-agcn_amd/ops.py
@@ -96,6 +96,31 @@
     return e[2] if hit else None
 
 
+_BN_BWD_FUSED = []
+
+
+def bn_bwd_fused_enabled():
+    if not _BN_BWD_FUSED:
+        _BN_BWD_FUSED.append(os.environ.get('AGCN_BN_BWD_FUSED', '1') != '0')
+    return _BN_BWD_FUSED[0]
+
+
+_BN_PART = [None]
+BN_BWD_STATS = {'fused': 0, 'reduce': 0}
+_BN_PART_DIRECT_ROWS = 256
+
+
+def _note_bn_part(t, part, key):
+    _BN_PART[0] = (weakref.ref(t), t._version, part, weakref.ref(key))
+
+
+def _take_bn_part(t, key):
+    e, _BN_PART[0] = _BN_PART[0], None
+    if e is not None and e[0]() is t and t._version == e[1] and e[3]() is key:
+        return e[2]
+    return None
+
+
 def conv_out_frames(T, taps, stride, pad=None):
     pad = (taps - 1) // 2 if pad is None else pad
     return (T + 2 * pad - taps) // stride + 1
@@ -122,12 +147,25 @@
 
 
 def conv_bwd_data(dy, w, x_shape, stride=1, out=None, accumulate=False, add1=None, mask1=None, add2=None,
-                  mask2=None, dy_amax=None, pad=None):
+                  mask2=None, dy_amax=None, pad=None, bn_sums=None):
     N, Cin, T, V = x_shape
     Cout, _, taps, _ = w.shape
     pad = (taps - 1) // 2 if pad is None else pad
     dx = out if out is not None else _empty(x_shape, dy)
     ws, nb = _conv_ws(Cin, Cout, T, V, taps, stride, dy, pad)
+    if bn_sums is not None and bn_bwd_fused_enabled():
+        y1, y2, bits = bn_sums
+        rows = _L().agcn_tconv_bwd_data_bn_rows(Cin, Cout, T, V, taps, stride, pad)
+        if rows > 0 and tuple(y1.shape) == tuple(x_shape) and bits is not None:
+            part = _empty((N * rows, Cin, 3), dy)
+            rc = _L().agcn_tconv_bwd_data_bn(_lib.ptr(dy), _lib.ptr(w), _lib.ptr(dx), int(accumulate), _lib.ptr(add1),
+                                            _lib.ptr(mask1), _lib.ptr(add2), _lib.ptr(mask2), ws.data_ptr(), nb, N, Cin,
+                                            Cout, T, V, taps, stride, pad, _lib.ptr(dy_amax), _lib.ptr(y1), _lib.ptr(y2),
+                                            _lib.ptr_bits(bits), _lib.ptr(part), N * rows, _lib.stream())
+            if rc != ERR_UNSUPPORTED:
+                _lib.check(rc, "agcn_tconv_bwd_data_bn")
+                _note_bn_part(dx, part, y1)
+                return dx
     _lib.check(_L().agcn_tconv_bwd_data(_lib.ptr(dy), _lib.ptr(w), _lib.ptr(dx), int(accumulate), _lib.ptr(add1),
                                         _lib.ptr(mask1), _lib.ptr(add2), _lib.ptr(mask2), ws.data_ptr(), nb, N, Cin,
                                         Cout, T, V, taps, stride, pad, _lib.ptr(dy_amax), _lib.stream()),
@@ -649,11 +687,15 @@
         return dy1, dg1, db1, dy2, dg2, db2
     N, C, T, V = y1.shape
     S = st1.S
+    slab = _take_bn_part(dout, y1)
+    if S > 1 or slab is None or slab.shape[1] != C or mask is None or mask.dtype != torch.int32:
+        slab = None
+    BN_BWD_STATS['fused' if slab is not None else 'reduce'] += 1
     if S > 1:
         N, C = N // S, C * S
         gamma1 = gamma1.repeat(S)
         gamma2 = gamma2.repeat(S) if gamma2 is not None else None
-    part = _empty((N * C * 3,), y1)
+    part = _empty((N * C * 3,), y1) if slab is None else None
     coef = _empty((6 * C,), y1)
     dy1 = torch.empty_like(y1)
     dg1, db1 = _empty((C,), y1), _empty((C,), y1)
@@ -663,7 +705,22 @@
         dg2, db2 = _empty((C,), y1), _empty((C,), y1)
     mbits = int(mask is not None and mask.dtype == torch.int32)
     mptr = _lib.ptr_bits(mask) if mbits else _lib.ptr(mask)
-    if sync is None and amax_out is not None:
+    if slab is not None:
+        nrows = slab.shape[0]
+        if sync is not None:
+            slab, nrows = _allreduce_sum(_colsum(slab, nrows, 3 * C), sync), 1
+            total, pscale = float(gcount) if gcount is not None else float(N * T * V * sync.world), 1.0 / sync.world
+        else:
+            if nrows > _BN_PART_DIRECT_ROWS:
+                slab, nrows = _colsum(slab, nrows, 3 * C), 1
+            total, pscale = float(N) * float(T * V), 1.0
+        _lib.check(_L().agcn_bn_bwd_apply_ex(
+            _lib.ptr(slab), nrows, total, pscale, _lib.ptr(dout), mptr, mbits, _lib.ptr(y1),
+            _lib.ptr(gamma1), _lib.ptr(st1.mean), _lib.ptr(st1.invstd), _lib.ptr(y2), _lib.ptr(gamma2),
+            _lib.ptr(st2.mean) if st2 else None, _lib.ptr(st2.invstd) if st2 else None, _lib.ptr(coef), _lib.ptr(dy1),
+            _lib.ptr(dg1), _lib.ptr(db1), _lib.ptr(dy2), _lib.ptr(dg2), _lib.ptr(db2), _lib.ptr(amax_out), N, C, T * V,
+            _lib.stream()), "agcn_bn_bwd_apply")
+    elif sync is None and amax_out is not None:
         _lib.check(_L().agcn_bn_bwd_reduce(_lib.ptr(dout), mptr, mbits, _lib.ptr(y1), _lib.ptr(y2),
                                            _lib.ptr(part), N, C, T * V, _lib.stream()), "agcn_bn_bwd_reduce")
         _lib.check(_L().agcn_bn_bwd_apply_ex(
@@ -869,7 +926,10 @@
     t_g_amax = getattr(c, 't_g_amax', None)
     dw = _side_run(lambda: conv_bwd_weight(dzpre, t_g, w.shape, t_stride, dz_amax, t_g_amax, pad=t_pad),
                    (dzpre, t_g, dz_amax, t_g_amax))
-    dg = conv_bwd_data(dzpre, w, c.t_g.shape, c.t_stride, dy_amax=dz_amax, pad=t_pad)
+    bn_sums = None
+    if getattr(c, 'g_out', None) is c.t_g and not c.g_bn1.eval and c.g_bn1.S == 1:
+        bn_sums = (c.g_ypre, c.g_dpre, c.g_bits)
+    dg = conv_bwd_data(dzpre, w, c.t_g.shape, c.t_stride, dy_amax=dz_amax, pad=t_pad, bn_sums=bn_sums)
     dwres = None
     if drpre is not None:
         t_resx = c.t_resx
diff --git a/include/agcn_hip.h b/include/agcn_hip.h
--- a/include/agcn_hip.h
+++ b/include/agcn_hip.h
@@ -87,6 +87,12 @@
                         const float* mask1, const float* add2, const float* mask2, void* workspace,
                         size_t workspace_bytes, int N, int Cin, int Cout, int T, int V, int taps, int stride, int pad,
                         const float* dy_absmax, void* stream);
+int agcn_tconv_bwd_data_bn_rows(int Cin, int Cout, int T, int V, int taps, int stride, int pad);
+int agcn_tconv_bwd_data_bn(const float* dy, const float* w, float* dx, int accumulate, const float* add1,
+                           const float* mask1, const float* add2, const float* mask2, void* workspace,
+                           size_t workspace_bytes, int N, int Cin, int Cout, int T, int V, int taps, int stride, int pad,
+                           const float* dy_absmax, const float* bn_y1, const float* bn_y2, const void* bn_bits,
+                           float* bn_part, int bn_rows, void* stream);
 size_t agcn_tconv_bwd_weight_workspace(int N, int Cin, int Cout, int T, int V, int taps, int stride, int pad);
 int agcn_tconv_bwd_weight(const float* dy, const float* x, float* dw, void* workspace, size_t workspace_bytes, int N,
                           int Cin, int Cout, int T, int V, int taps, int stride, int pad, const float* dy_absmax,
```

Measured after the change: 1056 clips/s (median of 6 runs). No clear change (+0.3%).
